# ZooMEISTER/vickers-hardness-Unet

Hardware: AMD Instinct MI355X
Metric: 512x512 images/sec (train fwd+bwd) (higher is better)
Workload: dtype bf16

## Files before the change

### include/vk_unet.h

```cpp
#ifndef VK_UNET_H
#define VK_UNET_H

#include <stddef.h>
#include <stdint.h>

#ifdef __cplusplus
extern "C" {
#endif

#define VK_ABI_VERSION 1
#define VK_STATS_REPLICAS 32

typedef enum { VK_F32 = 0, VK_BF16 = 1, VK_F16 = 2 } vk_dtype;

enum { VK_OK = 0, VK_ERR_ARG = -1, VK_ERR_STATE = -2, VK_ERR_UNSUPPORTED = -3 };

int vk_version(void);
const char* vk_last_error_string(void);
int vk_has_gfx950_code(void);
int vk_probe_mfma_rate(int iters, int waves_per_simd, float* sink, double* flops_out, void* stream);
int vk_set_reserved_cus(int n);
int vk_debug_hold_cus(int workgroups, int threads, int lds_bytes, int microseconds, const void* traffic, size_t traffic_bytes,
                      float* sink, void* stream);

int vk_debug_set_stamp_buffer(void* device_buffer);
int vk_prof_enable(int on);
int vk_prof_collect(char* buf, size_t buflen);


typedef struct {
  const void* ptr;
  int C;
  int up;
  const float* scale;
  const float* shift;
  int relu;
} vk_src;

typedef struct {
  vk_dtype dtype;
  int N, H, W;
  int Ho, Wo;
  int K;
  int R, S, stride, pad;
  int transposed;
  vk_src src0, src1;
} vk_conv_desc;

int vk_conv_fwd(const vk_conv_desc* d, const void* w, void* y, void* y1, int split_k1, int accumulate,
                double* stats, void* stream);

int vk_conv_dgrad_pool2(const vk_conv_desc* d, const void* w, void* y_half, void* y1, int split_k1, int accumulate,
                        void* stream);

int vk_halo_pack(vk_dtype dtype, int rows, int red, const void* src, void* dst, void* stream);
int vk_conv_uses_halo_pack(const vk_conv_desc* d);
int vk_conv_fwd_packed(const vk_conv_desc* d, const void* w_halo, void* y, void* y1, int split_k1, int accumulate, double* stats,
                       void* stream);

#define VK_SPLITK_WORKSPACE_BYTES (32u << 20)
int vk_conv_fwd_splitk(const vk_conv_desc* d, const void* w_halo, void* y, void* workspace, size_t workspace_bytes, void* stream);

typedef struct {
  const void* z;
  const float* scale;
  const float* shift;
  double* sums;
  const void* mask;
  int accumulate;
} vk_bnr;

int vk_conv_dgrad_fused(const vk_conv_desc* d, const void* w, void* y, void* y1, int split_k1, int pool2, const vk_bnr* bnr,
                        void* stream);

int vk_conv1x1_fwd(const vk_conv_desc* d, const void* w, void* y, int accumulate, double* stats, void* stream);
int vk_conv1x1_wgrad(const vk_conv_desc* d, const void* dz, float* dw, void* workspace, size_t workspace_bytes, void* stream);

int vk_stem_fwd(vk_dtype dtype, int N, int H, int W, const void* x4, const void* wp, void* y, double* stats,
                void* stream);

#define VK_WGRAD_WORKSPACE_BYTES (64u << 20)
int vk_conv_wgrad(const vk_conv_desc* d, const void* dz, float* dw, void* workspace, size_t workspace_bytes, void* stream);
#define VK_WGRAD_BATCH_TABLE_BYTES (128u << 10)
int vk_conv_wgrad_batch_supports(const vk_conv_desc* d);
int vk_conv_wgrad_batch(const vk_conv_desc* descs, const void* const* dz, float* const* dw, int n, int workgroups, void* tables,
                        size_t tables_bytes, void* workspace, size_t workspace_bytes, void* stream);
int vk_stem_wgrad(vk_dtype dtype, int N, int H, int W, const void* x4, const void* dz, float* dw_krsc3, void* workspace,
                  size_t workspace_bytes, void* stream);
int vk_stem_wgrad_bn(vk_dtype dtype, int N, int H, int W, const void* x4, const void* g, const void* z, const float* coef_abc,
                     float* dw_krsc3, void* workspace, size_t workspace_bytes, void* stream);
int vk_conv_bwd_onepass(const vk_conv_desc* d_fwd, const void* g, const void* z, const float* coef_abc, const void* w_dgrad, void* y,
                        const vk_bnr* bnr, float* dw, void* workspace, size_t workspace_bytes, void* stream);
int vk_stem_dgrad(vk_dtype dtype, int N, int H, int W, const void* g, const void* z, const float* coef_abc, const float* w_krsc3,
                  float* dx, void* stream);

typedef struct {
  int h, w;
  int src_stride;
  int size;
  int nh, nw;
  int top, left;
  int pad_value;
} vk_letterbox_desc;

int vk_letterbox_preprocess(const vk_letterbox_desc* d, const uint8_t* bgr, float* x_nchw, void* stream);
int vk_letterbox_postprocess_mask(const vk_letterbox_desc* d, const float* logits, float thresh, uint8_t* mask_hw, void* stream);
int vk_letterbox_postprocess_prob(const vk_letterbox_desc* d, const float* logits, float* prob_hw, void* stream);
int vk_letterbox_postprocess_labels(const vk_letterbox_desc* d, int C, const float* logits, uint8_t* labels_hw, void* stream);
int vk_letterbox_postprocess_mask_multi(const vk_letterbox_desc* d, int C, const float* logits, float thresh, uint8_t* masks_chw,
                                        void* stream);
int vk_letterbox_postprocess_prob_multi(const vk_letterbox_desc* d, int C, int mode, const float* logits, float* probs_chw, void* stream);

#define VK_TILE_MAX_ORIGINS 64
#define VK_TILE_MAX_SIDE 4096
#define VK_BLEND_PROB 0
#define VK_BLEND_LOGIT 1
typedef struct {
  int h, w;
  int src_stride;
  int T;
  int overlap;
  int ny, nx;
  int ys[VK_TILE_MAX_ORIGINS], xs[VK_TILE_MAX_ORIGINS];
  int view_mask;
  int pad_value;
  int C;
} vk_tile_desc;

int vk_tile_preprocess(const vk_tile_desc* d, const uint8_t* bgr, float* x, void* stream);
int vk_tile_blend(const vk_tile_desc* d, int mode, const float* logits, float thresh, float* out_chw, uint8_t* mask_chw, void* stream);

typedef struct {
  int h, w;
  float bin_thresh;
  int morph_kernel;
  int open_iter;
  int close_iter;
  int min_area;
  int max_components;
} vk_geom_desc;

typedef struct {
  int label;
  int area;
  int box[8];
  float cx, cy;
  float rw, rh;
  float ux, uy;
  int hull_n;
  int reserved;
  double d1, d2, d_mean;
} vk_geom_det;

int64_t vk_geom_workspace_bytes(const vk_geom_desc* d, int batch);
int vk_geom_minarearect(const vk_geom_desc* d, int batch, const float* prob, uint8_t* clean, vk_geom_det* dets, int* counts,
                        void* workspace, size_t workspace_bytes, void* stream);

typedef struct {
  int label;
  int area;
  int box[8];
  float cx, cy;
  int valid;
  int branch;
  int n_candidates;
  int contour_n;
  int hull_n;
  int flags;
  double quality;
  double d1, d2, d_mean;
} vk_geom_quad;

int vk_geom_quadrilateral(const vk_geom_desc* d, int fit_outset_px, int batch, const float* prob, uint8_t* clean, vk_geom_quad* dets,
                          int* counts, void* workspace, size_t workspace_bytes, void* stream);

typedef struct {
  int d4;
  int rotate;
  float cos_a, sin_a;
  int photo;
  float alpha, beta;
  int blur_ksize;
  float noise_scale;
  uint32_t noise_seed;
  int clahe_limit;
} vk_aug_params;

#define VK_AUG_TABLE_INTS (256 + 4097 + 4097)
size_t vk_augment_workspace_bytes(int n, int size);

int vk_letterbox_u8(const vk_letterbox_desc* d, const uint8_t* bgr, uint8_t* rgb_sq, void* stream);
int vk_letterbox_mask_u8(const vk_letterbox_desc* d, const uint8_t* mask_hw, uint8_t* mask_sq, void* stream);
int vk_augment_batch(int n, int size, int n_items, const uint8_t* images_rgb, const uint8_t* masks, const int* index_dev,
                     const vk_aug_params* params_host, void* params_dev, const int* color_tables, void* workspace,
                     size_t workspace_bytes, float* x, float* y, void* stream);

int vk_input_transform(vk_dtype dtype, int N, int H, int W, const float* x, void* x4, void* stream);

int vk_bn_finalize(int C, int train, const double* stats, double count, const float* gamma, const float* beta,
                   float* running_mean, float* running_var, float eps, float momentum, float* scale, float* shift,
                   float* save_mean, float* save_invstd, void* stream);

int vk_bn_relu_maxpool(vk_dtype dtype, int N, int H, int W, int C, const void* z, const float* scale,
                       const float* shift, void* pooled, uint8_t* argmax, void* stream);
int vk_maxpool_bwd(vk_dtype dtype, int N, int H, int W, int C, const void* dpool, const uint8_t* argmax, void* dy,
                   void* stream);
int vk_maxpool_bwd_bn_reduce(vk_dtype dtype, int N, int H, int W, int C, const void* dpool, const uint8_t* argmax, const void* z,
                             const float* scale, const float* shift, void* dy, double* sums, void* stream);

int vk_bn_add_relu(vk_dtype dtype, size_t pixels, int C, const void* z, const float* scale, const float* shift,
                   const void* res, const float* rscale, const float* rshift, void* out, void* stream);

int vk_bn_bwd_reduce(vk_dtype dtype, size_t pixels, int C, const void* dy, const void* z, int mask_mode,
                     const float* scale, const float* shift, const void* mask_src, double* sums, void* stream);
int vk_bn_bwd_coeffs(int C, const double* sums, double count, const float* gamma, const float* save_mean,
                     const float* save_invstd, float* dgamma, float* dbeta, float* coef_abc, void* stream);
int vk_bn_bwd_apply(vk_dtype dtype, size_t pixels, int C, const void* dy, const void* z, int mask_mode,
                    const float* scale, const float* shift, const void* mask_src, const float* coef_abc, void* dz,
                    void* g_out, int g_accumulate, void* stream);
int vk_bn_bwd_coeffs_frozen(int C, const double* sums, const float* gamma, const float* running_mean, const float* running_invstd,
                            float* dgamma, float* dbeta, float* coef_abc, void* stream);
int vk_bn_bwd_apply_fused(vk_dtype dtype, size_t pixels, int C, const void* dy, const void* z, int mask_mode,
                          const float* scale, const float* shift, const void* mask_src, const double* sums, double count,
                          const float* gamma, const float* save_mean, const float* save_invstd, float* dgamma, float* dbeta,
                          void* dz, void* g_out, int g_accumulate, void* stream);

// ... 178 lines not shown
```

### vickers-hardness-unet_amd/_lib.py

```python
from __future__ import annotations

import ctypes as C
import os
import subprocess
from pathlib import Path

PKG_DIR = Path(__file__).resolve().parent
LIB_PATH = Path(os.environ["VK_LIB"]) if os.environ.get("VK_LIB") else PKG_DIR / "libvkunet.so"
CSRC = PKG_DIR / "csrc"

VK_F32, VK_BF16, VK_F16 = 0, 1, 2
VK_LOSS_BINARY, VK_LOSS_MULTILABEL, VK_LOSS_MULTICLASS = 0, 1, 2
VK_ENC_RESNET18, VK_ENC_RESNET34, VK_ENC_RESNET50 = 18, 34, 50
VK_ADAMW_MAX_GROUPS = 8
VK_NORM_L2, VK_NORM_INF = 0, 1
VK_TILE_MAX_ORIGINS, VK_TILE_MAX_SIDE = 64, 4096
VK_BLEND_PROB, VK_BLEND_LOGIT = 0, 1


class VkError(RuntimeError):
    pass


class vk_src(C.Structure):
    _fields_ = [("ptr", C.c_void_p), ("C", C.c_int), ("up", C.c_int), ("scale", C.c_void_p),
                ("shift", C.c_void_p), ("relu", C.c_int)]


class vk_conv_desc(C.Structure):
    _fields_ = [("dtype", C.c_int), ("N", C.c_int), ("H", C.c_int), ("W", C.c_int), ("Ho", C.c_int),
                ("Wo", C.c_int), ("K", C.c_int), ("R", C.c_int), ("S", C.c_int), ("stride", C.c_int),
                ("pad", C.c_int), ("transposed", C.c_int), ("src0", vk_src), ("src1", vk_src)]


class vk_bnr(C.Structure):
    _fields_ = [("z", C.c_void_p), ("scale", C.c_void_p), ("shift", C.c_void_p), ("sums", C.c_void_p), ("mask", C.c_void_p),
                ("accumulate", C.c_int)]


class vk_letterbox_desc(C.Structure):
    _fields_ = [("h", C.c_int), ("w", C.c_int), ("src_stride", C.c_int), ("size", C.c_int), ("nh", C.c_int),
                ("nw", C.c_int), ("top", C.c_int), ("left", C.c_int), ("pad_value", C.c_int)]


class vk_tile_desc(C.Structure):
    _fields_ = [("h", C.c_int), ("w", C.c_int), ("src_stride", C.c_int), ("T", C.c_int), ("overlap", C.c_int), ("ny", C.c_int),
                ("nx", C.c_int), ("ys", C.c_int * VK_TILE_MAX_ORIGINS), ("xs", C.c_int * VK_TILE_MAX_ORIGINS), ("view_mask", C.c_int),
                ("pad_value", C.c_int), ("C", C.c_int)]


class vk_geom_desc(C.Structure):
    _fields_ = [("h", C.c_int), ("w", C.c_int), ("bin_thresh", C.c_float), ("morph_kernel", C.c_int), ("open_iter", C.c_int),
                ("close_iter", C.c_int), ("min_area", C.c_int), ("max_components", C.c_int)]


class vk_geom_det(C.Structure):
    _fields_ = [("label", C.c_int), ("area", C.c_int), ("box", C.c_int * 8), ("cx", C.c_float), ("cy", C.c_float),
                ("rw", C.c_float), ("rh", C.c_float), ("ux", C.c_float), ("uy", C.c_float), ("hull_n", C.c_int),
                ("reserved", C.c_int), ("d1", C.c_double), ("d2", C.c_double), ("d_mean", C.c_double)]


class vk_geom_quad(C.Structure):
    _fields_ = [("label", C.c_int), ("area", C.c_int), ("box", C.c_int * 8), ("cx", C.c_float), ("cy", C.c_float),
                ("valid", C.c_int), ("branch", C.c_int), ("n_candidates", C.c_int), ("contour_n", C.c_int), ("hull_n", C.c_int),
                ("flags", C.c_int), ("quality", C.c_double), ("d1", C.c_double), ("d2", C.c_double), ("d_mean", C.c_double)]


class vk_aug_params(C.Structure):
    _fields_ = [("d4", C.c_int), ("rotate", C.c_int), ("cos_a", C.c_float), ("sin_a", C.c_float), ("photo", C.c_int),
                ("alpha", C.c_float), ("beta", C.c_float), ("blur_ksize", C.c_int), ("noise_scale", C.c_float),
                ("noise_seed", C.c_uint32), ("clahe_limit", C.c_int)]


class vk_seg_loss_cfg(C.Structure):
    _fields_ = [("struct_size", C.c_uint32), ("mode", C.c_int32), ("terms", C.c_uint32), ("has_ignore", C.c_int32),
                ("ignore_index", C.c_int32), ("w_pix", C.c_float), ("w_focal", C.c_float), ("w_dice", C.c_float),
                ("w_jaccard", C.c_float), ("w_tversky", C.c_float), ("pix_smooth", C.c_float), ("pix_denom_valid", C.c_int32),
                ("has_pos_weight", C.c_int32), ("pos_weight", C.c_float * 16), ("focal_has_alpha", C.c_int32),
                ("focal_alpha", C.c_float), ("focal_gamma", C.c_float),
                ("dice_smooth", C.c_float), ("dice_eps", C.c_float), ("dice_log", C.c_int32), ("dice_classes", C.c_uint32),
                ("jaccard_smooth", C.c_float), ("jaccard_eps", C.c_float), ("jaccard_log", C.c_int32), ("jaccard_classes", C.c_uint32),
                ("tversky_smooth", C.c_float), ("tversky_eps", C.c_float), ("tversky_log", C.c_int32), ("tversky_classes", C.c_uint32),
                ("tversky_alpha", C.c_float), ("tversky_beta", C.c_float), ("tversky_gamma", C.c_float),
                ("w_mcc", C.c_float), ("mcc_eps", C.c_float)]


class vk_lovasz_cfg(C.Structure):
    _fields_ = [("struct_size", C.c_uint32), ("mode", C.c_int32), ("per_image", C.c_int32), ("has_ignore", C.c_int32),
                ("ignore_index", C.c_int32)]


class vk_adamw_group(C.Structure):
    _fields_ = [("lr", C.c_float), ("beta1", C.c_float), ("beta2", C.c_float), ("eps", C.c_float), ("weight_decay", C.c_float)]


class vk_unet_config(C.Structure):
    _fields_ = [("N", C.c_int), ("size", C.c_int), ("dtype", C.c_int), ("training", C.c_int), ("width", C.c_int)]


class vk_tensor_info(C.Structure):
    _fields_ = [("name", C.c_char * 96), ("kind", C.c_int), ("dims", C.c_int * 4), ("ndim", C.c_int),
                ("offset", C.c_int64), ("numel", C.c_int64)]


vp, ci, cf, cd, sz, i64 = C.c_void_p, C.c_int, C.c_float, C.c_double, C.c_size_t, C.c_int64
P = C.POINTER

SIGNATURES = {
    "vk_version": (ci, []),
    "vk_last_error_string": (C.c_char_p, []),
    "vk_has_gfx950_code": (ci, []),
    "vk_probe_mfma_rate": (ci, [ci, ci, vp, P(C.c_double), vp]),
    "vk_set_reserved_cus": (ci, [ci]),
    "vk_debug_hold_cus": (ci, [ci, ci, ci, ci, vp, sz, vp, vp]),
    "vk_debug_set_stamp_buffer": (ci, [vp]),
    "vk_prof_enable": (ci, [ci]),
    "vk_prof_collect": (ci, [C.c_char_p, sz]),
    "vk_conv_fwd": (ci, [P(vk_conv_desc), vp, vp, vp, ci, ci, vp, vp]),
    "vk_conv_dgrad_pool2": (ci, [P(vk_conv_desc), vp, vp, vp, ci, ci, vp]),
    "vk_conv_dgrad_fused": (ci, [P(vk_conv_desc), vp, vp, vp, ci, ci, P(vk_bnr), vp]),
    "vk_head_bwd_fused": (ci, [ci, ci, ci, ci, P(vk_src), vp, vp, vp, vp, vp, P(vk_bnr), vp, sz, vp]),
    "vk_halo_pack": (ci, [ci, ci, ci, vp, vp, vp]),
    "vk_conv_uses_halo_pack": (ci, [P(vk_conv_desc)]),
    "vk_conv_fwd_packed": (ci, [P(vk_conv_desc), vp, vp, vp, ci, ci, vp, vp]),
    "vk_conv_fwd_splitk": (ci, [P(vk_conv_desc), vp, vp, vp, sz, vp]),
    "vk_stem_fwd": (ci, [ci, ci, ci, ci, vp, vp, vp, vp, vp]),
    "vk_conv_wgrad": (ci, [P(vk_conv_desc), vp, vp, vp, sz, vp]),
    "vk_conv1x1_fwd": (ci, [P(vk_conv_desc), vp, vp, ci, vp, vp]),
    "vk_conv1x1_wgrad": (ci, [P(vk_conv_desc), vp, vp, vp, sz, vp]),
    "vk_conv_wgrad_batch_supports": (ci, [P(vk_conv_desc)]),
    "vk_conv_wgrad_batch": (ci, [P(vk_conv_desc), P(vp), P(vp), ci, ci, vp, sz, vp, sz, vp]),
    "vk_stem_wgrad": (ci, [ci, ci, ci, ci, vp, vp, vp, vp, sz, vp]),
    "vk_stem_wgrad_bn": (ci, [ci, ci, ci, ci, vp, vp, vp, vp, vp, vp, sz, vp]),
    "vk_conv_bwd_onepass": (ci, [P(vk_conv_desc), vp, vp, vp, vp, vp, P(vk_bnr), vp, vp, sz, vp]),
    "vk_stem_dgrad": (ci, [ci, ci, ci, ci, vp, vp, vp, vp, vp, vp]),
    "vk_letterbox_preprocess": (ci, [P(vk_letterbox_desc), vp, vp, vp]),
    "vk_letterbox_postprocess_mask": (ci, [P(vk_letterbox_desc), vp, cf, vp, vp]),
    "vk_letterbox_postprocess_prob": (ci, [P(vk_letterbox_desc), vp, vp, vp]),
    "vk_letterbox_postprocess_labels": (ci, [P(vk_letterbox_desc), ci, vp, vp, vp]),
    "vk_letterbox_postprocess_mask_multi": (ci, [P(vk_letterbox_desc), ci, vp, cf, vp, vp]),
    "vk_letterbox_postprocess_prob_multi": (ci, [P(vk_letterbox_desc), ci, ci, vp, vp, vp]),
    "vk_tile_preprocess": (ci, [P(vk_tile_desc), vp, vp, vp]),
    "vk_tile_blend": (ci, [P(vk_tile_desc), ci, vp, cf, vp, vp, vp]),
    "vk_geom_workspace_bytes": (i64, [P(vk_geom_desc), ci]),
    "vk_geom_minarearect": (ci, [P(vk_geom_desc), ci, vp, vp, vp, vp, vp, sz, vp]),
    "vk_geom_quadrilateral": (ci, [P(vk_geom_desc), ci, ci, vp, vp, vp, vp, vp, sz, vp]),
    "vk_letterbox_u8": (ci, [P(vk_letterbox_desc), vp, vp, vp]),
    "vk_letterbox_mask_u8": (ci, [P(vk_letterbox_desc), vp, vp, vp]),
    "vk_augment_workspace_bytes": (C.c_size_t, [ci, ci]),
    "vk_augment_batch": (ci, [ci, ci, ci, vp, vp, vp, P(vk_aug_params), vp, vp, vp, C.c_size_t, vp, vp, vp]),
    "vk_input_transform": (ci, [ci, ci, ci, ci, vp, vp, vp]),
    "vk_bn_finalize": (ci, [ci, ci, vp, cd, vp, vp, vp, vp, cf, cf, vp, vp, vp, vp, vp]),
    "vk_bn_relu_maxpool": (ci, [ci, ci, ci, ci, ci, vp, vp, vp, vp, vp, vp]),
    "vk_maxpool_bwd": (ci, [ci, ci, ci, ci, ci, vp, vp, vp, vp]),
    "vk_maxpool_bwd_bn_reduce": (ci, [ci, ci, ci, ci, ci, vp, vp, vp, vp, vp, vp, vp, vp]),
    "vk_bn_add_relu": (ci, [ci, sz, ci, vp, vp, vp, vp, vp, vp, vp, vp]),
    "vk_bn_bwd_reduce": (ci, [ci, sz, ci, vp, vp, ci, vp, vp, vp, vp, vp]),
    "vk_bn_bwd_coeffs": (ci, [ci, vp, cd, vp, vp, vp, vp, vp, vp, vp]),
    "vk_bn_bwd_coeffs_frozen": (ci, [ci, vp, vp, vp, vp, vp, vp, vp, vp]),
    "vk_bn_bwd_apply": (ci, [ci, sz, ci, vp, vp, ci, vp, vp, vp, vp, vp, vp, ci, vp]),
    "vk_bn_bwd_apply_fused": (ci, [ci, sz, ci, vp, vp, ci, vp, vp, vp, vp, cd, vp, vp, vp, vp, vp, vp, vp, ci, vp]),
    "vk_upsample2x_bwd": (ci, [ci, ci, ci, ci, ci, vp, vp, ci, vp]),
    "vk_head_fwd": (ci, [ci, ci, ci, ci, P(vk_src), vp, vp, vp, vp]),
    "vk_dec4_tail_eval": (ci, [ci, ci, ci, ci, P(vk_src), vp, vp, vp, vp, vp, vp, vp, vp, vp, vp]),
    "vk_head_bwd": (ci, [ci, ci, ci, ci, P(vk_src), vp, vp, vp, vp, vp, vp, sz, vp]),
    "vk_bce_dice_loss": (ci, [sz, vp, vp, vp, vp, vp, cf, cf, cf, vp]),
    "vk_head_fwd_multi": (ci, [ci, ci, ci, ci, ci, P(vk_src), vp, vp, vp, vp]),
    "vk_head_multi_workspace_bytes": (sz, [ci]),
    "vk_head_bwd_multi": (ci, [ci, ci, ci, ci, ci, P(vk_src), vp, vp, vp, vp, vp, P(vk_bnr), vp, sz, vp]),
    "vk_multi_loss_workspace_bytes": (sz, [ci, ci, ci]),
    "vk_multilabel_loss": (ci, [ci, ci, ci, vp, vp, vp, sz, vp, vp, cf, cf, cf, vp]),
    "vk_multiclass_loss": (ci, [ci, ci, ci, vp, vp, vp, sz, vp, vp, cf, cf, cf, vp]),
    "vk_seg_loss_cfg_size": (sz, []),
    "vk_seg_loss_workspace_bytes": (sz, [ci, ci, ci]),
    "vk_seg_loss": (ci, [P(vk_seg_loss_cfg), ci, ci, ci, vp, vp, vp, sz, vp, vp, cf, vp]),
    "vk_lovasz_cfg_size": (sz, []),
    "vk_lovasz_workspace_bytes": (sz, [P(vk_lovasz_cfg), ci, ci, ci]),
    "vk_lovasz_loss": (ci, [P(vk_lovasz_cfg), ci, ci, ci, vp, vp, vp, sz, vp, vp, cf, ci, vp]),
    "vk_lovasz_flat_workspace_bytes": (sz, [ci, i64]),
    "vk_lovasz_flat": (ci, [vp, vp, ci, i64, vp, sz, vp, vp, vp, vp]),
    "vk_seg_metrics_workspace_bytes": (C.c_size_t, [ci]),
    "vk_seg_metrics": (ci, [ci, sz, vp, vp, ci, cf, cf, vp, sz, vp, vp]),
    "vk_seg_metrics_multi_workspace_bytes": (sz, [ci, ci]),
    "vk_seg_metrics_multi": (ci, [ci, ci, ci, sz, vp, vp, ci, cf, cf, vp, sz, vp, vp, vp, vp]),
    "vk_adamw_step": (ci, [sz, vp, vp, vp, vp, cf, cf, cf, cf, cf, ci, cf, vp, vp, ci, vp]),
    "vk_amp_check_inf": (ci, [sz, vp, vp, vp]),
    "vk_amp_unscale_check": (ci, [sz, vp, vp, vp, vp]),
    "vk_adamw_step_amp": (ci, [sz, vp, vp, vp, vp, cf, cf, cf, cf, cf, vp, cf, vp, vp, vp, vp, ci, vp]),
    "vk_adamw_segment_blocks": (ci, [ci, P(i64), P(C.c_int32), ci]),
    "vk_adamw_step_amp_segments": (ci, [ci, vp, ci, vp, vp, vp, vp, vp, cf, cf, cf, cf, cf, vp, cf, vp, vp, vp, vp]),
    "vk_adamw_step_groups": (ci, [ci, vp, vp, ci, vp, vp, vp, vp, vp, ci, P(vk_adamw_group), vp, cf, vp, vp, vp, vp, vp]),
    "vk_grad_norm_segments": (ci, [ci, vp, ci, vp, vp, ci, cf, cf, vp, vp, vp]),
    "vk_unet_create": (ci, [P(vk_unet_config), P(vp)]),
    "vk_unet_create_ex": (ci, [P(vk_unet_config), ci, P(vp)]),
    "vk_unet_num_classes": (ci, [vp]),
    "vk_unet_create_enc": (ci, [P(vk_unet_config), ci, ci, P(vp)]),
    "vk_unet_encoder": (ci, [vp]),
    "vk_unet_destroy": (None, [vp]),
    "vk_unet_set_side_stream": (ci, [vp, ci]),
    "vk_unet_num_tensors": (ci, [vp]),
    "vk_unet_tensor_info": (ci, [vp, ci, P(vk_tensor_info)]),
    "vk_unet_param_numel": (i64, [vp]),
    "vk_unet_buffer_numel": (i64, [vp]),
    "vk_unet_workspace_bytes": (i64, [vp]),
    "vk_unet_num_buckets": (ci, [vp]),
    "vk_unet_bucket_range": (ci, [vp, ci, P(i64), P(i64)]),
    "vk_unet_bind": (ci, [vp, vp, vp, vp, vp, vp, sz]),
    "vk_unet_refresh_weights": (ci, [vp, vp]),
    "vk_unet_forward": (ci, [vp, vp, vp, ci, vp]),
    "vk_unet_loss": (ci, [vp, vp, vp, vp, cf, cf, cf, vp]),
    "vk_unet_loss_ex": (ci, [vp, ci, vp, vp, vp, cf, cf, cf, vp]),
    "vk_unet_loss_cfg": (ci, [vp, P(vk_seg_loss_cfg), vp, vp, vp, cf, vp]),
    "vk_unet_loss_lovasz": (ci, [vp, P(vk_seg_loss_cfg), P(vk_lovasz_cfg), cf, vp, vp, vp, sz, vp, cf, vp]),
    "vk_unet_backward": (ci, [vp, vp, ci, ci, vp]),
    "vk_unet_set_trainable": (ci, [vp, P(C.c_uint8), ci]),
    "vk_unet_set_bn_frozen": (ci, [vp, P(C.c_uint8), ci]),
    "vk_unet_set_input_grad": (ci, [vp, vp]),
    "vk_unet_zero_grad": (ci, [vp, vp]),
    "vk_unet_debug_tensor": (ci, [vp, C.c_char_p, P(vp), P(ci * 4)]),
    "vk_comm_unique_id": (ci, [vp]),
    "vk_comm_init": (ci, [ci, ci, vp, P(vp)]),
    "vk_comm_world": (ci, [vp]),
    "vk_allreduce_bucket": (ci, [vp, vp, sz, vp]),
    "vk_comm_broadcast": (ci, [vp, vp, sz, ci, vp]),
    "vk_comm_destroy": (ci, [vp]),
}

_lib = None


def build(force: bool = False, verbose: bool = False) -> Path:
    srcs = list(CSRC.glob("*.hip")) + list(CSRC.glob("*.h")) + [PKG_DIR.parent / "include" / "vk_unet.h"]
    if not force and LIB_PATH.exists() and all(LIB_PATH.stat().st_mtime >= s.stat().st_mtime for s in srcs):
        return LIB_PATH
    hipcc = os.environ.get("HIPCC", "/opt/rocm/bin/hipcc")
    if not Path(hipcc).exists():
        raise VkError(f"hipcc not found at {hipcc}; cannot build libvkunet.so")
    cmd = ["make", "-C", str(CSRC), f"-j{min(4, os.cpu_count() or 1)}", f"HIPCC={hipcc}"]
    r = subprocess.run(cmd, capture_output=True, text=True)
    if verbose:
        print(r.stdout[-2000:], r.stderr[-2000:])
    if r.returncode != 0 or not LIB_PATH.exists():
        raise VkError("building libvkunet.so failed:\n" + r.stdout[-3000:] + r.stderr[-3000:])
    return LIB_PATH


def lib():
    global _lib
    if _lib is not None:
        return _lib
    if not LIB_PATH.exists():
        raise VkError(f"{LIB_PATH} is missing: build it with __graft_entry__.build() "
                      f"(make -C {CSRC}); this package has no CPU fallback")
    try:
        L = C.CDLL(str(LIB_PATH))
    except OSError as e:
        raise VkError(f"cannot load {LIB_PATH}: {e}") from e
    for name, (res, args) in SIGNATURES.items():
        fn = getattr(L, name, None)
        if fn is None:
            raise VkError(f"{LIB_PATH} does not export {name}")
        fn.restype = res
        fn.argtypes = args
    if L.vk_version() != 1:
        raise VkError("libvkunet.so ABI version mismatch")
    _lib = L
    return L


def check(rc: int, what: str = "") -> None:
    if rc != 0:
        msg = lib().vk_last_error_string().decode(errors="replace")
        kind = "argument/state error" if rc < 0 else f"hipError {rc}"
        raise VkError(f"{what or 'libvkunet'}: {kind}: {msg}")


def dtype_code(dt) -> int:
    import torch
# ... 21 lines not shown
```

### vickers-hardness-unet_amd/csrc/conv_halo.hip

```cpp
#include <stdlib.h>
#include <string.h>

#include <string>
#include <type_traits>

#include "vk_common.h"

#ifdef VK_STAMP
#define VK_T(var) { __builtin_amdgcn_sched_barrier(0); const unsigned long long t_ = __builtin_amdgcn_s_memtime(); __builtin_amdgcn_s_waitcnt(0xC07F); __builtin_amdgcn_sched_barrier(0); var = t_; }
#else
#define VK_T(var)
#endif

namespace vk {

struct HaloSrc {
  const void* ptr;
  const float* scale;
  const float* shift;
  int C, up, relu;
  uint32_t bytes;
};

#ifndef VK_EPI_BATCH_READS
#define VK_EPI_BATCH_READS 1
#endif
#ifndef VK_COLP_DEFER_STATS
#define VK_COLP_DEFER_STATS 1
#endif
#ifndef VK_COLQ_ILV
#define VK_COLQ_ILV 1
#endif
#ifndef VK_COLQ_DIAG
#define VK_COLQ_DIAG 0
#endif
#ifndef VK_COLQ_PRE
#define VK_COLQ_PRE 1
#endif
struct HaloParams {
  HaloSrc s0, s1;
  const void* w;
  uint32_t w_bytes;
  void* y0;
  void* y1;
  int ld0, ld1, split;
  double* stats;
  int N, H, W, K, C, flip, accumulate, pool2;
  int Hi, Wi;
  int tiles_x, tiles_y, nchunks;
  unsigned long long* stamps;
  int kyn;
  int ksplit;
  size_t slab_bytes;
  float* slab;
  int dbg;
  const void* bnr_z;
  const float* bnr_scale;
  const float* bnr_shift;
  double* bnr_sums;
  const void* bnr_mask;
};

template <typename T, int TH, int BN, int WGM, int WGN>
struct HaloCfg {
  using Tr = ElemTraits<T>;
  static constexpr int EB = Tr::kBytes;
  static constexpr int VE = Tr::kVec;
  static constexpr int CK = 64 / EB;
  static constexpr int HW_ = 18, HH = TH + 2, HPIX = HH * HW_;
  static constexpr int APS = 96;
  static constexpr int A_BYTES = HPIX * APS;
  static constexpr int B_BYTES = 3 * BN * 64;
  static constexpr int NPV = (HPIX * 4 + 255) / 256;
  static constexpr int NBV = (3 * BN * 4 + 255) / 256;
  static constexpr int BM = TH * 16;
  static constexpr int WR = TH / WGM;
  static constexpr int WCH = BN / WGN;
  static constexpr int TP = WR, TC = WCH / 16;
  static constexpr int ESB = BN * EB + 16;
  static constexpr int EVPR = BN / VE;
  static constexpr int ERPP = 256 / EVPR;
  static constexpr int EPASS = BM / ERPP;
  static constexpr int RED_OFF = BM * ESB;
  static constexpr int MAIN = A_BYTES + 2 * B_BYTES;
  static constexpr int ESLOTS = (BN / VE > 16) ? 4 * 4 / (BN / VE / 16) : 4 * 4;
  static constexpr int EPI = RED_OFF + ESLOTS * BN * 2 * 4;
  static constexpr int SMEM = MAIN > EPI ? MAIN : EPI;
  static_assert(WGM * WGN == 4 && TH % WGM == 0 && BN % (16 * WGN) == 0, "wave layout");
  static_assert(EPASS >= 1, "epilogue mapping");
  static_assert(SMEM <= 160 * 1024, "main-loop / epilogue LDS image exceeds the 160 KiB of a CU");
};

__device__ __forceinline__ int swz(int row) { return ((row >> 2) & 1) << 1; }

__device__ __forceinline__ int halo_group(int tid) {
  const int g = tid >> 2;
  return (g & ~3) | ((g & 1) << 1) | ((g >> 1) & 1);
}


template <typename T, int TH, int BN, int TP, int TC, int NT = 256, bool PRE = false, int OS = 1>
__device__ __forceinline__ void halo_epilogue(char* smem, f32x4_t (&acc)[TC][TP], const HaloParams& p, int n, int y0, int x0, int n0,
                                              int wrow0, int wch0, int py = 0, int px = 0, double* defer = nullptr) {
  using Tr = ElemTraits<T>;
  constexpr int EB = Tr::kBytes, VE = Tr::kVec;
  constexpr int BM = TH * 16;
  constexpr int ESB = BN * EB + 16;
  constexpr int EVPR = BN / VE, ERPP = NT / EVPR, EPASS = BM / ERPP, NW = NT / 64;
  constexpr int RED_OFF = BM * ESB;
  static_assert(BM % ERPP == 0 && EVPR <= 64, "epilogue mapping");
  const int tid = threadIdx.x, lane = tid & 63, wave = tid >> 6;
  const int li = lane & 15, kg = lane >> 4;

  const int e_row = tid / EVPR;
  const int e_vec = (EVPR == 16 && EB == 2) ? (((tid & 15) + ((e_row & 1) ? 15 : 0)) & 15) : tid % EVPR;
  const int col0 = n0 + e_vec * VE;
  const bool col_ok = col0 < p.K;
  char* yb = (char*)p.y0;
  int ld = p.ld0, colx = col0;
  bool first_part = true;
  if (p.split > 0 && col0 >= p.split) { yb = (char*)p.y1; ld = p.ld1; colx = col0 - p.split; first_part = false; }
  float s1[VE], s2[VE];
#pragma unroll
  for (int j = 0; j < VE; ++j) { s1[j] = 0.f; s2[j] = 0.f; }
  const bool bnr = p.bnr_z != nullptr && first_part && col_ok;
  const bool ext_mask = p.bnr_mask != nullptr;
  float bsc[VE], bsh[VE];
  if (bnr && !ext_mask) {
#pragma unroll
    for (int j = 0; j < VE; ++j) { bsc[j] = p.bnr_scale[colx + j]; bsh[j] = p.bnr_shift[colx + j]; }
  }
  auto finish = [&](float (&f)[VE], size_t elem_off, const u32x4_t* pre_old, const u32x4_t* pre_z, const u32x4_t* pre_m = nullptr) {
    u32x4_t* gp = reinterpret_cast<u32x4_t*>(yb + elem_off * EB);
    if (p.accumulate) {
      float o[VE];
      Vec16<T>::unpack(pre_old ? *pre_old : *gp, o);
#pragma unroll
      for (int j = 0; j < VE; ++j) f[j] += o[j];
    }
    u32x4_t v = Vec16<T>::pack(f);
    Vec16<T>::unpack(v, f);
    if (bnr) {
      float zf[VE];
      Vec16<T>::unpack(pre_z ? *pre_z : *reinterpret_cast<const u32x4_t*>((const char*)p.bnr_z + elem_off * EB), zf);
      if (ext_mask) {
        float mf[VE];
        Vec16<T>::unpack(pre_m ? *pre_m : *reinterpret_cast<const u32x4_t*>((const char*)p.bnr_mask + elem_off * EB), mf);
#pragma unroll
        for (int j = 0; j < VE; ++j)
          if (!(mf[j] > 0.f)) f[j] = 0.f;
      } else {
#pragma unroll
        for (int j = 0; j < VE; ++j)
          if (!(fmaf(zf[j], bsc[j], bsh[j]) > 0.f)) f[j] = 0.f;
      }
#pragma unroll
      for (int j = 0; j < VE; ++j) {
        s1[j] += f[j];
        s2[j] += f[j] * zf[j];
      }
      v = Vec16<T>::pack(f);
    } else {
#pragma unroll
      for (int j = 0; j < VE; ++j) { s1[j] += f[j]; s2[j] += f[j] * f[j]; }
    }
    *gp = v;
  };
  constexpr bool PRE_M = PRE && NT == 512;
  u32x4_t oldv[PRE ? EPASS : 1], zv[PRE ? EPASS : 1], mv[PRE_M ? EPASS : 1];
  constexpr bool EARLY = PRE && NT == 512;
  auto request_pre = [&]() {
    if (!(PRE && (p.accumulate || bnr) && !(p.pool2 && first_part))) return;
#pragma unroll
    for (int ps = 0; ps < (PRE ? EPASS : 0); ++ps) {
      const int row = e_row + ps * ERPP;
      const int y = OS * (y0 + (row >> 4)) + py, x = OS * (x0 + (row & 15)) + px;
      oldv[ps] = u32x4_t{0, 0, 0, 0};
      zv[ps] = u32x4_t{0, 0, 0, 0};
      if (PRE_M) mv[ps] = u32x4_t{0, 0, 0, 0};
      if (y < p.H && x < p.W && col_ok) {
        const size_t eoff = (((size_t)n * p.H + y) * p.W + x) * ld + colx;
        if (p.accumulate) oldv[ps] = *reinterpret_cast<const u32x4_t*>(yb + eoff * EB);
        if (bnr) zv[ps] = *reinterpret_cast<const u32x4_t*>((const char*)p.bnr_z + eoff * EB);
        if (PRE_M && bnr && ext_mask) mv[ps] = *reinterpret_cast<const u32x4_t*>((const char*)p.bnr_mask + eoff * EB);
      }
    }
  };
  if (EARLY) request_pre();
#pragma unroll
  for (int a = 0; a < TC; ++a)
#pragma unroll
    for (int b = 0; b < TP; ++b) {
      const int ch = wch0 + a * 16 + kg * 4;
      const int px = (wrow0 + b) * 16 + li;
      char* dst = smem + px * ESB + ch * EB;
      if (EB == 4) {
        *reinterpret_cast<f32x4_t*>(dst) = acc[a][b];
      } else {
        float f[8] = {acc[a][b][0], acc[a][b][1], acc[a][b][2], acc[a][b][3], 0.f, 0.f, 0.f, 0.f};
        const u32x4_t pk = Vec16<T>::pack(f);
        *reinterpret_cast<u32x2_t*>(dst) = u32x2_t{pk[0], pk[1]};
      }
    }
  __syncthreads();
  if (!EARLY) request_pre();

  if (p.pool2 && first_part) {
    const int Hh = p.H >> 1, Wh = p.W >> 1;
    for (int pr = e_row; pr < (TH / 2) * 8; pr += ERPP) {
      const int py = pr >> 3, px = pr & 7;
      const int y = (y0 >> 1) + py, x = (x0 >> 1) + px;
      if (y < Hh && x < Wh && col_ok) {
        float f[VE];
// ... 173 lines not shown
    const bool first = c < p.s0.C;
    const HaloSrc& sd = first ? p.s0 : p.s1;
    const int cl = (first ? c : c - p.s0.C) + hv * VE;
    aff = sd.scale != nullptr;
    relu = sd.relu != 0;
    if (aff) {
#pragma unroll
      for (int j = 0; j < VE; j += 4) {
        const f32x4_t s4 = *reinterpret_cast<const f32x4_t*>(sd.scale + cl + j);
        const f32x4_t h4 = *reinterpret_cast<const f32x4_t*>(sd.shift + cl + j);
#pragma unroll
        for (int e = 0; e < 4; ++e) { sc[j + e] = s4[e]; sh[j + e] = h4[e]; }
      }
    }
    const bool up = sd.up != 0;
#pragma unroll
    for (int i = 0; i < NPV; ++i) {
      const int pix = up ? h_half[i] : h_full[i];
      const uint32_t off = (uint32_t)(pix * sd.C + cl) * (uint32_t)EB;
      if (first) areg[i] = buf_load16(rs0, pix >= 0 ? off : kOOB);
      else areg[i] = buf_load16(rs1, pix >= 0 ? off : kOOB);
    }
  };

  auto store_halo = [&]() {
#pragma unroll
    for (int i = 0; i < NPV; ++i) {
      const int hp = hgrp + i * 64;
      if (hp >= HPIX) continue;
      u32x4_t v = areg[i];
      if (aff) {
        v = AffineRelu<T>::run(v, sc, sh, relu);
        if (h_full[i] < 0) v = u32x4_t{0, 0, 0, 0};
      }
      *reinterpret_cast<u32x4_t*>(Abuf + hp * APS + hv * 16) = v;
    }
  };

  auto load_b = [&](u32x4_t (&breg)[NBV], int stage) {
    const int cc = stage / 3, r = stage - cc * 3;
#pragma unroll
    for (int i = 0; i < NBV; ++i) {
      const int tap = p.flip ? 8 - (3 * r + b_s[i]) : 3 * r + b_s[i];
      const uint32_t base = (uint32_t)(cc * 9 + tap) * slab_bytes + (uint32_t)n0 * 64u;
      breg[i] = buf_load16(rsw, b_toff[i] >= 0 ? base + (uint32_t)b_toff[i] : kOOB);
    }
  };
  auto store_b = [&](const u32x4_t (&breg)[NBV], int buf) {
    char* B = Bbuf + buf * Cfg::B_BYTES;
#pragma unroll
    for (int i = 0; i < NBV; ++i)
      if (b_toff[i] >= 0) *reinterpret_cast<u32x4_t*>(B + b_s[i] * (BN * 64) + b_toff[i]) = breg[i];
  };

  const int wrow0 = (wave / WGN) * Cfg::WR;
  const int wch0 = (wave % WGN) * Cfg::WCH;
  f32x4_t acc[TC][TP];
#pragma unroll
  for (int a = 0; a < TC; ++a)
#pragma unroll
    for (int b = 0; b < TP; ++b) acc[a][b] = f32x4_t{0.f, 0.f, 0.f, 0.f};
  const int li = lane & 15, kg = lane >> 4;
  const char* const a_lane = Abuf + (wrow0 * 18 + li) * APS + kg * 16;
  const int b_lane = (wch0 + li) * 64 + ((kg ^ swz(li)) << 4);

  auto compute = [&](int bbuf, int r) {
    const char* A = a_lane + r * (18 * APS);
    const char* B = Bbuf + bbuf * Cfg::B_BYTES + b_lane;
    u32x4_t wf[2][TC], xf[2][TP];
#pragma unroll
    for (int a = 0; a < TC; ++a) wf[0][a] = *reinterpret_cast<const u32x4_t*>(B + (a * 16) * 64);
#pragma unroll
    for (int b = 0; b < TP; ++b) xf[0][b] = *reinterpret_cast<const u32x4_t*>(A + (b * 18) * APS);
#pragma unroll
    for (int s = 0; s < 3; ++s) {
      if (s < 2) {
#pragma unroll
        for (int a = 0; a < TC; ++a) wf[(s + 1) & 1][a] = *reinterpret_cast<const u32x4_t*>(B + ((s + 1) * BN + a * 16) * 64);
#pragma unroll
        for (int b = 0; b < TP; ++b) xf[(s + 1) & 1][b] = *reinterpret_cast<const u32x4_t*>(A + (b * 18 + s + 1) * APS);
      }
#pragma unroll
      for (int a = 0; a < TC; ++a)
#pragma unroll
        for (int b = 0; b < TP; ++b) acc[a][b] = Mma<T>::run(wf[s & 1][a], xf[s & 1][b], acc[a][b]);
    }
    constexpr int NR = TC + TP, NM = TC * TP * (sizeof(T) == 4 ? 4 : 1);
    __builtin_amdgcn_sched_group_barrier(0x100, NR, 0);
    __builtin_amdgcn_sched_group_barrier(0x100, NR, 0);
    __builtin_amdgcn_sched_group_barrier(0x008, NM, 0);
    __builtin_amdgcn_sched_group_barrier(0x100, NR, 0);
    __builtin_amdgcn_sched_group_barrier(0x008, NM, 0);
    __builtin_amdgcn_sched_group_barrier(0x008, NM, 0);
  };

#ifdef VK_STAMP
  unsigned long long t_begin;
  VK_T(t_begin)
#endif
  const int nst = p.nchunks * 3;
  load_halo(0);
  load_b(breg0, 0);
  store_halo();
  store_b(breg0, 0);
  if (nst > 1) load_b(breg1, 1);
  __syncthreads();

#ifdef VK_STAMP
  unsigned long long tk_load = 0, tk_comp = 0, tk_store = 0, tk_bar = 0;
#endif
  auto stage = [&](int st, u32x4_t (&ld_regs)[NBV], const u32x4_t (&st_regs)[NBV]) {
    const int cc = st / 3, r = st - cc * 3;
    const bool next_chunk = cc + 1 < p.nchunks;
#ifdef VK_STAMP
    unsigned long long t0, t1, t2, t3, t4;
#endif
    VK_T(t0)
    if (st + 2 < nst) load_b(ld_regs, st + 2);
    if (r == 0 && next_chunk) load_halo(cc + 1);
    VK_T(t1)
    compute(st & 1, r);
    VK_T(t2)
    if (r == 2 && next_chunk) {
      __syncthreads();
      store_halo();
    }
    if (st + 1 < nst) store_b(st_regs, (st + 1) & 1);
    VK_T(t3)
    __syncthreads();
    VK_T(t4)
#ifdef VK_STAMP
    tk_load += t1 - t0; tk_comp += t2 - t1; tk_store += t3 - t2; tk_bar += t4 - t3;
#endif
  };
  for (int st = 0; st < nst; st += 2) {
    stage(st, breg0, breg1);
    if (st + 1 < nst) stage(st + 1, breg1, breg0);
  }

#ifdef VK_STAMP
  unsigned long long te0, te1;
  VK_T(te0)
#endif
  halo_epilogue<T, TH, BN, TP, TC>(smem, acc, p, n, y0, x0, n0, wrow0, wch0);
#ifdef VK_STAMP
  VK_T(te1)
  if (p.stamps && lane == 0) {
    unsigned long long* o = p.stamps + ((size_t)(blockIdx.y * gridDim.x + blockIdx.x) * 4 + wave) * 8;
    o[0] = tk_load; o[1] = tk_comp; o[2] = tk_store; o[3] = tk_bar; o[4] = te1 - te0; o[5] = te0 - t_begin; o[6] = te1 - t_begin; o[7] = nst;
  }
#endif
}

template <typename T, int TH, int BN, int WGM, int WGN, bool ADB, int STR = 1>
struct ColCfg {
  using Tr = ElemTraits<T>;
  static constexpr int EB = Tr::kBytes;
  static constexpr int VE = Tr::kVec;
  static constexpr int CK = 64 / EB;
  static constexpr int NW = WGM * WGN, NT = 64 * NW;
  static constexpr int HH = STR == 1 ? TH + 2 : 2 * TH + 1;
  static constexpr int HWI = STR == 1 ? 18 : 33;
  static constexpr int RS = STR == 1 ? 18 : 34;
  static constexpr int HPIX = HH * HWI;
  static constexpr int APS = 96;
  static constexpr int A_BYTES = HH * RS * APS;
  static constexpr int NA = ADB ? 2 : 1;
  static constexpr int B_BYTES = 3 * BN * 64;
  static constexpr int NPV = (HPIX * 4 + NT - 1) / NT;
  static constexpr int NPIECE = 3 * BN / 16;
  static constexpr int BM = TH * 16;
  static constexpr int TP = TH / WGM, TC = BN / WGN / 16;
  static constexpr int NX = STR * (TP - 1) + 3;
  static constexpr int ESB = BN * EB + 16;
  static constexpr int NB = (BN <= 64 && STR == 1) ? 3 : 2;
  static constexpr int MAIN = NA * A_BYTES + NB * B_BYTES;
  static constexpr int ESLOTS = (BN / VE > 16) ? NW * 4 / (BN / VE / 16) : NW * 4;
  static constexpr int EPI = BM * ESB + ESLOTS * BN * 2 * 4;
  static constexpr int SMEM = MAIN > EPI ? MAIN : EPI;
  static_assert(TH % WGM == 0 && BN % (16 * WGN) == 0 && (NW == 4 || NW == 8), "wave layout");
  static_assert(STR == 1 || STR == 2, "stride");
  static_assert(SMEM <= 160 * 1024, "main-loop / epilogue LDS image exceeds the 160 KiB of a CU");
  static_assert(EPI >= BM * ESB + ESLOTS * BN * 8, "epilogue partial-sum slots must fit behind the output tile");
};

template <typename T, int TH, int BN, int WGM, int WGN, bool ADB, int MINW, int STR = 1>
__global__ __launch_bounds__(64 * WGM * WGN, MINW) void conv3x3_col_kernel(const HaloParams p) {
  using Cfg = ColCfg<T, TH, BN, WGM, WGN, ADB, STR>;
  constexpr int EB = Cfg::EB, VE = Cfg::VE, CK = Cfg::CK, HPIX = Cfg::HPIX, NPV = Cfg::NPV, NT = Cfg::NT, NW = Cfg::NW;
  constexpr int TP = Cfg::TP, TC = Cfg::TC, APS = Cfg::APS, NPIECE = Cfg::NPIECE, RS = Cfg::RS, HWI = Cfg::HWI, NX = Cfg::NX;
  typedef __attribute__((address_space(3))) void lds_void;

  extern __shared__ __attribute__((aligned(16))) char smem[];
  char* const Abuf = smem;
  char* const Bbuf = smem + Cfg::NA * Cfg::A_BYTES;
  const int tid = threadIdx.x, lane = tid & 63;
  const int wave = __builtin_amdgcn_readfirstlane(tid >> 6);

  int bt = blockIdx.x;
  int ky = blockIdx.y;
  if (p.kyn > 0) {
    const int j = bt >> 3;
    ky = j % p.kyn;
    bt = (bt & 7) * (int)((gridDim.x / p.kyn) >> 3) + j / p.kyn;
  } else if (p.kyn < 0) {
    const int kn = -p.kyn, xcd = bt & 7;
    ky = xcd % kn;
    bt = (xcd / kn) * (int)(gridDim.x >> 3) + (bt >> 3);
  } else if ((gridDim.x & 7) == 0) {
    bt = (bt & 7) * (int)(gridDim.x >> 3) + (bt >> 3);
  }
  const int tx = bt % p.tiles_x;
  bt /= p.tiles_x;
  const int ty = bt % p.tiles_y;
  const int n = bt / p.tiles_y;
  const int y0 = ty * TH, x0 = tx * 16;
  const int n0 = ky * BN;

  const __amdgpu_buffer_rsrc_t rs0 = make_rsrc(p.s0.ptr, p.s0.bytes);
  const __amdgpu_buffer_rsrc_t rs1 = make_rsrc(p.s1.ptr ? p.s1.ptr : p.s0.ptr, p.s1.ptr ? p.s1.bytes : 0u);
  const __amdgpu_buffer_rsrc_t rsw = make_rsrc(p.w, p.w_bytes);

  const int hv = tid & 3;
  const int hgrp = halo_group(tid);
  int h_full[NPV], h_half[NPV];
  const int Hh = p.Hi >> 1, Wh = p.Wi >> 1;
#pragma unroll
  for (int i = 0; i < NPV; ++i) {
    const int hp = hgrp + i * (NT / 4);
    const int hy = hp / HWI, hx = hp - hy * HWI;
    const int y = STR * y0 - 1 + hy, x = STR * x0 - 1 + hx;
    const bool ok = hp < HPIX && (unsigned)y < (unsigned)p.Hi && (unsigned)x < (unsigned)p.Wi;
    h_full[i] = ok ? (n * p.Hi + y) * p.Wi + x : -1;
    h_half[i] = ok ? (n * Hh + (y >> 1)) * Wh + (x >> 1) : -1;
  }
  u32x4_t areg[NPV];
  float sc[VE], sh[VE];
  bool aff = false, relu = false;

  auto load_halo = [&](int cc) {
    const int c = cc * CK;
    const bool first = c < p.s0.C;
    const HaloSrc& sd = first ? p.s0 : p.s1;
    const int cl = (first ? c : c - p.s0.C) + hv * VE;
    aff = sd.scale != nullptr;
    relu = sd.relu != 0;
    if (aff) {
#pragma unroll
      for (int j = 0; j < VE; j += 4) {
        const f32x4_t s4 = *reinterpret_cast<const f32x4_t*>(sd.scale + cl + j);
        const f32x4_t h4 = *reinterpret_cast<const f32x4_t*>(sd.shift + cl + j);
#pragma unroll
        for (int e = 0; e < 4; ++e) { sc[j + e] = s4[e]; sh[j + e] = h4[e]; }
      }
    }
    const bool up = STR == 1 && sd.up != 0;
#pragma unroll
    for (int i = 0; i < NPV; ++i) {
      const int pix = up ? h_half[i] : h_full[i];
      const uint32_t off = (uint32_t)(pix * sd.C + cl) * (uint32_t)EB;
      if (first) areg[i] = buf_load16(rs0, pix >= 0 ? off : kOOB);
      else areg[i] = buf_load16(rs1, pix >= 0 ? off : kOOB);
    }
  };
  auto store_halo = [&](char* A) {
#pragma unroll
    for (int i = 0; i < NPV; ++i) {
      const int hp = hgrp + i * (NT / 4);
      if (hp >= HPIX) continue;
      u32x4_t v = areg[i];
      if (aff) {
        v = AffineRelu<T>::run(v, sc, sh, relu);
        if (h_full[i] < 0) v = u32x4_t{0, 0, 0, 0};
      }
      int slot = hp;
      if (STR == 2) {
        const int hy = hp / HWI, hx = hp - hy * HWI;
        slot = hy * RS + (hx & 1) * 17 + (hx >> 1);
      }
      *reinterpret_cast<u32x4_t*>(A + slot * APS + hv * 16) = v;
    }
  };

  const uint32_t slab_bytes = (uint32_t)p.K * 64u;
  const uint32_t lane16 = (uint32_t)lane * 16u;
  auto dma_b = [&](int cc, int s, int buf) {
#pragma unroll
    for (int i = 0; i < (NPIECE + NW - 1) / NW; ++i) {
      const int pc = wave + i * NW;
      if (NPIECE % NW == 0 || pc < NPIECE) {
        const int r = pc / (BN / 16), sub = pc - r * (BN / 16);
        const int tap = p.flip ? 8 - (3 * r + s) : 3 * r + s;
        const uint32_t goff = (uint32_t)(cc * 9 + tap) * slab_bytes + (uint32_t)(n0 + sub * 16) * 64u;
        char* dst = Bbuf + buf * Cfg::B_BYTES + (r * BN + sub * 16) * 64;
        __builtin_amdgcn_raw_ptr_buffer_load_lds(rsw, (lds_void*)dst, 16, lane16, goff, 0, 0);
      }
    }
  };

  const int wrow0 = (wave / WGN) * TP;
  const int wch0 = (wave % WGN) * (TC * 16);
  f32x4_t acc[TC][TP];
#pragma unroll
  for (int a = 0; a < TC; ++a)
#pragma unroll
    for (int b = 0; b < TP; ++b) acc[a][b] = f32x4_t{0.f, 0.f, 0.f, 0.f};
  const int li = lane & 15, kg = lane >> 4;
  const int a_lane = (STR * wrow0 * RS + li) * APS + kg * 16;
  const int b_lane = (wch0 + li) * 64 + ((kg ^ swz(li)) << 4);

  auto compute = [&](const char* A, const char* B) {
    u32x4_t X[NX], W[3][TC];
#pragma unroll
    for (int h = 0; h < NX; ++h) X[h] = *reinterpret_cast<const u32x4_t*>(A + h * (RS * APS));
#pragma unroll
    for (int r = 0; r < 3; ++r)
#pragma unroll
      for (int a = 0; a < TC; ++a) W[r][a] = *reinterpret_cast<const u32x4_t*>(B + (r * BN + a * 16) * 64);
#pragma unroll
    for (int r = 0; r < 3; ++r)
#pragma unroll
      for (int a = 0; a < TC; ++a)
#pragma unroll
        for (int b = 0; b < TP; ++b) acc[a][b] = Mma<T>::run(W[r][a], X[STR * b + r], acc[a][b]);
    constexpr int NM = TC * TP * (sizeof(T) == 4 ? 4 : 1);
    __builtin_amdgcn_sched_group_barrier(0x100, NX + TC, 0);
    __builtin_amdgcn_sched_group_barrier(0x100, TC, 0);
    __builtin_amdgcn_sched_group_barrier(0x008, NM, 0);
    __builtin_amdgcn_sched_group_barrier(0x100, TC, 0);
    __builtin_amdgcn_sched_group_barrier(0x008, NM, 0);
    __builtin_amdgcn_sched_group_barrier(0x008, NM, 0);
  };

#ifdef VK_STAMP
  unsigned long long t_begin, t_pro, tk_load = 0, tk_comp = 0, tk_store = 0, tk_bar = 0;
  VK_T(t_begin)
#endif
  const int ksp = p.ksplit > 1 ? p.ksplit : 1;
  const int c_begin = (int)((long)p.nchunks * blockIdx.z / ksp), c_end = (int)((long)p.nchunks * (blockIdx.z + 1) / ksp);
  load_halo(c_begin);
  dma_b(c_begin, 0, 0);
  const bool one_chunk = Cfg::NB == 3 && c_end - c_begin == 1 && !p.dbg;
  if (one_chunk) {
    dma_b(c_begin, 1, 1);
    dma_b(c_begin, 2, 2);
  }
  store_halo(Abuf);
  __syncthreads();
  VK_T(t_pro)

  int st = 0;
  if (one_chunk) {
    const char* A = Abuf + a_lane;
#pragma unroll
    for (int s = 0; s < 3; ++s) compute(A + (STR == 1 ? s : (s & 1) * 17 + (s >> 1)) * APS, Bbuf + s * Cfg::B_BYTES + b_lane);
    __syncthreads();
    st = 3;
  }
  for (int cc = c_begin; cc < c_end && !one_chunk; ++cc) {
    const bool next_chunk = cc + 1 < c_end;
    const char* A = Abuf + (ADB ? ((cc - c_begin) & 1) * Cfg::A_BYTES : 0) + a_lane;
    char* const Anext = Abuf + (ADB ? ((cc - c_begin + 1) & 1) * Cfg::A_BYTES : 0);
#pragma unroll
    for (int s = 0; s < 3; ++s, ++st) {
#ifdef VK_STAMP
      unsigned long long t0, t1, t2, t3, t4;
#endif
      VK_T(t0)
      if (!(p.dbg & 2)) {
        if (s < 2) dma_b(cc, s + 1, (st + 1) & 1);
        else if (next_chunk) dma_b(cc + 1, 0, (st + 1) & 1);
      }
      if (s == 0 && next_chunk && !(p.dbg & 4)) load_halo(cc + 1);
      VK_T(t1)
      compute(A + (STR == 1 ? s : (s & 1) * 17 + (s >> 1)) * APS, Bbuf + (st & 1) * Cfg::B_BYTES + b_lane);
      VK_T(t2)
      if (ADB) {
        if (s == 1 && next_chunk && !(p.dbg & 4)) store_halo(Anext);
      } else {
        if (s == 2 && next_chunk && !(p.dbg & 4)) {
          __syncthreads();
          store_halo(Anext);
        }
      }
      VK_T(t3)
      if (!(p.dbg & 8)) __syncthreads();
      VK_T(t4)
#ifdef VK_STAMP
      tk_load += t1 - t0; tk_comp += t2 - t1; tk_store += t3 - t2; tk_bar += t4 - t3;
#endif
    }
  }
#ifdef VK_STAMP
  unsigned long long te0, te1;
  VK_T(te0)
#endif
  if (p.ksplit > 1) {
    float* sl = p.slab + (size_t)blockIdx.z * ((size_t)p.N * p.H * p.W * p.K);
#pragma unroll
    for (int a = 0; a < TC; ++a)
#pragma unroll
      for (int b = 0; b < TP; ++b) {
        const int y = y0 + wrow0 + b, x = x0 + li, ch = n0 + wch0 + a * 16 + kg * 4;
        if (y < p.H && x < p.W && ch < p.K) *reinterpret_cast<f32x4_t*>(sl + (((size_t)n * p.H + y) * p.W + x) * p.K + ch) = acc[a][b];
      }
    return;
  }
  halo_epilogue<T, TH, BN, TP, TC, NT, (BN <= 64 && TH == 16)>(smem, acc, p, n, y0, x0, n0, wrow0, wch0);
#ifdef VK_STAMP
  VK_T(te1)
  if (p.stamps && lane == 0) {
    unsigned long long* o = p.stamps + ((size_t)(blockIdx.y * gridDim.x + blockIdx.x) * NW + wave) * 8;
    o[0] = tk_load; o[1] = tk_comp; o[2] = tk_store; o[3] = tk_bar; o[4] = te1 - te0; o[5] = t_pro - t_begin; o[6] = te1 - t_begin; o[7] = st;
  }
#endif
}

template <typename T, int TH, int BN, int WGM, int WGN>
struct S2dCfg {
  using Tr = ElemTraits<T>;
  static constexpr int EB = Tr::kBytes, VE = Tr::kVec, CK = 64 / EB;
  static constexpr int NW = WGM * WGN, NT = 64 * NW;
  static constexpr int HH = TH + 1, RS = 17, HPIX = HH * RS, APS = 96;
  static constexpr int A_BYTES = HPIX * APS;
  static constexpr int B_BYTES = 3 * BN * 64;
  static constexpr int NPV = (HPIX * 4 + NT - 1) / NT;
  static constexpr int NPIECE = 3 * BN / 16;
  static constexpr int BM = TH * 16;
  static constexpr int TP = TH / WGM, TC = BN / WGN / 16;
  static constexpr int ESB = BN * EB + 16;
  static constexpr int MAIN = 2 * A_BYTES + 2 * B_BYTES;
  static constexpr int ESLOTS = (BN / VE > 16) ? NW * 4 / (BN / VE / 16) : NW * 4;
  static constexpr int EPI = BM * ESB + ESLOTS * BN * 2 * 4;
  static constexpr int SMEM = MAIN > EPI ? MAIN : EPI;
  static_assert(TH % WGM == 0 && BN % (16 * WGN) == 0 && NW == 8, "wave layout");
  static_assert(4 * TP * TC <= 32, "accumulator budget (four parity classes)");
  static_assert(SMEM <= 160 * 1024, "LDS image exceeds the 160 KiB of a CU");
};

template <typename T, int TH, int BN, int WGM, int WGN>
__global__ __launch_bounds__(64 * WGM * WGN, 1) void conv3x3_s2dg_kernel(const HaloParams p) {
  using Cfg = S2dCfg<T, TH, BN, WGM, WGN>;
  constexpr int EB = Cfg::EB, VE = Cfg::VE, CK = Cfg::CK, HPIX = Cfg::HPIX, NPV = Cfg::NPV, NT = Cfg::NT, NW = Cfg::NW;
  constexpr int TP = Cfg::TP, TC = Cfg::TC, APS = Cfg::APS, NPIECE = Cfg::NPIECE, RS = Cfg::RS;
  typedef __attribute__((address_space(3))) void lds_void;

  extern __shared__ __attribute__((aligned(16))) char smem[];
  char* const Abuf = smem;
  char* const Bbuf = smem + 2 * Cfg::A_BYTES;
  const int tid = threadIdx.x, lane = tid & 63;
  const int wave = __builtin_amdgcn_readfirstlane(tid >> 6);

  int bt = blockIdx.x;
  const int ky = blockIdx.y;
  if ((gridDim.x & 7) == 0) bt = (bt & 7) * (int)(gridDim.x >> 3) + (bt >> 3);
  const int tx = bt % p.tiles_x;
  bt /= p.tiles_x;
  const int ty = bt % p.tiles_y;
  const int n = bt / p.tiles_y;
  const int y0 = ty * TH, x0 = tx * 16;
  const int n0 = ky * BN;

  const __amdgpu_buffer_rsrc_t rs0 = make_rsrc(p.s0.ptr, p.s0.bytes);
  const __amdgpu_buffer_rsrc_t rsw = make_rsrc(p.w, p.w_bytes);

  const int hv = tid & 3;
  const int hgrp = halo_group(tid);
  int h_full[NPV];
#pragma unroll
  for (int i = 0; i < NPV; ++i) {
    const int hp = hgrp + i * (NT / 4);
    const int hy = hp / RS, hx = hp - hy * RS;
    const int y = y0 + hy, x = x0 + hx;
    const bool ok = hp < HPIX && y < p.Hi && x < p.Wi;
    h_full[i] = ok ? (n * p.Hi + y) * p.Wi + x : -1;
  }
  u32x4_t areg[NPV];
  auto load_halo = [&](int cc) {
    const int cl = cc * CK + hv * VE;
#pragma unroll
    for (int i = 0; i < NPV; ++i) {
      const uint32_t off = (uint32_t)(h_full[i] * p.s0.C + cl) * (uint32_t)EB;
      areg[i] = buf_load16(rs0, h_full[i] >= 0 ? off : kOOB);
    }
  };
  auto store_halo = [&](char* A) {
#pragma unroll
    for (int i = 0; i < NPV; ++i) {
      const int hp = hgrp + i * (NT / 4);
      if (hp < HPIX) *reinterpret_cast<u32x4_t*>(A + hp * APS + hv * 16) = areg[i];
    }
  };
  const uint32_t slab_bytes = (uint32_t)p.K * 64u;
  const uint32_t lane16 = (uint32_t)lane * 16u;
  auto dma_b = [&](int cc, int s, int buf) {
#pragma unroll
    for (int i = 0; i < (NPIECE + NW - 1) / NW; ++i) {
      const int pc = wave + i * NW;
      if (NPIECE % NW == 0 || pc < NPIECE) {
        const int r = pc / (BN / 16), sub = pc - r * (BN / 16);
        const uint32_t goff = (uint32_t)(cc * 9 + 3 * r + s) * slab_bytes + (uint32_t)(n0 + sub * 16) * 64u;
        char* dst = Bbuf + buf * Cfg::B_BYTES + (r * BN + sub * 16) * 64;
        __builtin_amdgcn_raw_ptr_buffer_load_lds(rsw, (lds_void*)dst, 16, lane16, goff, 0, 0);
      }
    }
  };

  const int wrow0 = (wave / WGN) * TP;
  const int wch0 = (wave % WGN) * (TC * 16);
  f32x4_t acc[4][TC][TP];
#pragma unroll
  for (int q = 0; q < 4; ++q)
#pragma unroll
    for (int a = 0; a < TC; ++a)
#pragma unroll
      for (int b = 0; b < TP; ++b) acc[q][a][b] = f32x4_t{0.f, 0.f, 0.f, 0.f};
  const int li = lane & 15, kg = lane >> 4;
  const int a_lane = (wrow0 * RS + li) * APS + kg * 16;
  const int b_lane = (wch0 + li) * 64 + ((kg ^ swz(li)) << 4);

  auto compute = [&](const char* A, const char* B, auto s_c) {
    constexpr int s = decltype(s_c)::value;
    u32x4_t X[TP + 1], W[3][TC];
#pragma unroll
    for (int h = 0; h < TP + 1; ++h) X[h] = *reinterpret_cast<const u32x4_t*>(A + ((s == 0 ? 1 : 0) + h * RS) * APS);
#pragma unroll
    for (int r = 0; r < 3; ++r)
#pragma unroll
      for (int a = 0; a < TC; ++a) W[r][a] = *reinterpret_cast<const u32x4_t*>(B + (r * BN + a * 16) * 64);
#pragma unroll
    for (int r = 0; r < 3; ++r) {
      constexpr int px = s != 1 ? 1 : 0;
      const int q = (r != 1 ? 2 : 0) + px, di = r == 0 ? 1 : 0;
#pragma unroll
      for (int a = 0; a < TC; ++a)
#pragma unroll
        for (int b = 0; b < TP; ++b) acc[q][a][b] = Mma<T>::run(W[r][a], X[b + di], acc[q][a][b]);
    }
  };

  load_halo(0);
  dma_b(0, 0, 0);
  store_halo(Abuf);
  __syncthreads();
  int st = 0;
  for (int cc = 0; cc < p.nchunks; ++cc) {
    const bool next_chunk = cc + 1 < p.nchunks;
    const char* A = Abuf + (cc & 1) * Cfg::A_BYTES + a_lane;
    char* const Anext = Abuf + ((cc + 1) & 1) * Cfg::A_BYTES;
    dma_b(cc, 1, (st + 1) & 1);
    if (next_chunk) load_halo(cc + 1);
    compute(A, Bbuf + (st & 1) * Cfg::B_BYTES + b_lane, std::integral_constant<int, 0>{});
    __syncthreads();
    ++st;
    dma_b(cc, 2, (st + 1) & 1);
    compute(A, Bbuf + (st & 1) * Cfg::B_BYTES + b_lane, std::integral_constant<int, 1>{});
    if (next_chunk) store_halo(Anext);
    __syncthreads();
    ++st;
    if (next_chunk) dma_b(cc + 1, 0, (st + 1) & 1);
    compute(A, Bbuf + (st & 1) * Cfg::B_BYTES + b_lane, std::integral_constant<int, 2>{});
    __syncthreads();
    ++st;
  }
#pragma unroll
  for (int q = 0; q < 4; ++q) {
    if (q) __syncthreads();
    halo_epilogue<T, TH, BN, TP, TC, NT, false, 2>(smem, acc[q], p, n, y0, x0, n0, wrow0, wch0, q >> 1, q & 1);
  }
}

template <typename T, int TH, int BN, int WGM, int WGN>
struct ColqCfg : ColCfg<T, TH, BN, WGM, WGN, true> {
  using Base = ColCfg<T, TH, BN, WGM, WGN, true>;
  static constexpr int MAIN = 2 * Base::A_BYTES + 3 * Base::B_BYTES;
  static constexpr int SMEM = MAIN > Base::EPI ? MAIN : Base::EPI;
  static constexpr int DMAW = Base::NPIECE / Base::NW;
  static_assert(Base::NPIECE % Base::NW == 0, "every wave must issue the same number of weight DMAs per stage (partial vmcnt wait)");
  static_assert(DMAW >= 1 && DMAW <= 15, "vmcnt immediate");
  static_assert(SMEM <= 160 * 1024, "LDS image exceeds the 160 KiB of a CU");
};

template <typename T, int TH, int BN, int WGM, int WGN>
__global__ __launch_bounds__(64 * WGM * WGN, 1) void conv3x3_colq_kernel(const HaloParams p) {
  using Cfg = ColqCfg<T, TH, BN, WGM, WGN>;
  constexpr int EB = Cfg::EB, VE = Cfg::VE, CK = Cfg::CK, HPIX = Cfg::HPIX, NPV = Cfg::NPV, NT = Cfg::NT, NW = Cfg::NW;
  constexpr int TP = Cfg::TP, TC = Cfg::TC, APS = Cfg::APS, NPIECE = Cfg::NPIECE;
  typedef __attribute__((address_space(3))) void lds_void;

  extern __shared__ __attribute__((aligned(16))) char smem[];
  char* const Abuf = smem;
  char* const Bbuf = smem + 2 * Cfg::A_BYTES;
  const int tid = threadIdx.x, lane = tid & 63;
  const int wave = __builtin_amdgcn_readfirstlane(tid >> 6);

  int bt = blockIdx.x;
  int ky = blockIdx.y;
  if (p.kyn > 0) {
    const int j = bt >> 3;
    ky = j % p.kyn;
    bt = (bt & 7) * (int)((gridDim.x / p.kyn) >> 3) + j / p.kyn;
  } else if (p.kyn < 0) {
    const int kn = -p.kyn, xcd = bt & 7;
    ky = xcd % kn;
    bt = (xcd / kn) * (int)(gridDim.x >> 3) + (bt >> 3);
  } else if ((gridDim.x & 7) == 0) {
    bt = (bt & 7) * (int)(gridDim.x >> 3) + (bt >> 3);
  }
  const int tx = bt % p.tiles_x;
  bt /= p.tiles_x;
  const int ty = bt % p.tiles_y;
  const int n = bt / p.tiles_y;
  const int y0 = ty * TH, x0 = tx * 16;
  const int n0 = ky * BN;

  const __amdgpu_buffer_rsrc_t rs0 = make_rsrc(p.s0.ptr, p.s0.bytes);
  const __amdgpu_buffer_rsrc_t rs1 = make_rsrc(p.s1.ptr ? p.s1.ptr : p.s0.ptr, p.s1.ptr ? p.s1.bytes : 0u);
  const __amdgpu_buffer_rsrc_t rsw = make_rsrc(p.w, p.w_bytes);

  const int hv = tid & 3;
  const int hgrp = halo_group(tid);
  int h_full[NPV], h_half[NPV];
  const int Hh = p.H >> 1, Wh = p.W >> 1;
#pragma unroll
  for (int i = 0; i < NPV; ++i) {
    const int hp = hgrp + i * (NT / 4);
    const int hy = hp / 18, hx = hp - hy * 18;
    const int y = y0 - 1 + hy, x = x0 - 1 + hx;
    const bool ok = hp < HPIX && (unsigned)y < (unsigned)p.H && (unsigned)x < (unsigned)p.W;
    h_full[i] = ok ? (n * p.H + y) * p.W + x : -1;
    h_half[i] = ok ? (n * Hh + (y >> 1)) * Wh + (x >> 1) : -1;
  }
  u32x4_t areg[NPV];
  float sc[VE], sh[VE];
  bool aff = false, relu = false;

  auto load_halo = [&](int cc) {
    const int c = cc * CK;
    const bool first = c < p.s0.C;
    const HaloSrc& sd = first ? p.s0 : p.s1;
    const int cl = (first ? c : c - p.s0.C) + hv * VE;
    aff = sd.scale != nullptr;
    relu = sd.relu != 0;
    if (aff) {
#pragma unroll
      for (int j = 0; j < VE; j += 4) {
        const f32x4_t s4 = *reinterpret_cast<const f32x4_t*>(sd.scale + cl + j);
        const f32x4_t h4 = *reinterpret_cast<const f32x4_t*>(sd.shift + cl + j);
#pragma unroll
        for (int e = 0; e < 4; ++e) { sc[j + e] = s4[e]; sh[j + e] = h4[e]; }
      }
    }
    const bool up = sd.up != 0;
#pragma unroll
    for (int i = 0; i < NPV; ++i) {
      const int pix = up ? h_half[i] : h_full[i];
      const uint32_t off = (uint32_t)(pix * sd.C + cl) * (uint32_t)EB;
      if (first) areg[i] = buf_load16(rs0, pix >= 0 ? off : kOOB);
      else areg[i] = buf_load16(rs1, pix >= 0 ? off : kOOB);
    }
  };
  auto store_halo = [&](char* A) {
#pragma unroll
    for (int i = 0; i < NPV; ++i) {
      const int hp = hgrp + i * (NT / 4);
      if (hp >= HPIX) continue;
      u32x4_t v = areg[i];
      if (aff) {
        v = (p.dbg & 32) ? AffineReluScalar<T>::run(v, sc, sh, relu) : AffineRelu<T>::run(v, sc, sh, relu);
        if (h_full[i] < 0) v = u32x4_t{0, 0, 0, 0};
      }
      *reinterpret_cast<u32x4_t*>(A + hp * APS + hv * 16) = v;
    }
  };

  const uint32_t slab_bytes = (uint32_t)p.K * 64u;
  const uint32_t lane16 = (uint32_t)lane * 16u;
  auto dma_b = [&](int cc, int s, uint32_t oob = 0u) {
#pragma unroll
    for (int i = 0; i < ((VK_COLQ_DIAG & 1) ? 1 : Cfg::DMAW); ++i) {
      const int pc = wave + i * NW;
      const int r = pc / (BN / 16), sub = pc - r * (BN / 16);
      const int tap = p.flip ? 8 - (3 * r + s) : 3 * r + s;
      const uint32_t goff = (uint32_t)(cc * 9 + tap) * slab_bytes + (uint32_t)(n0 + sub * 16) * 64u;
      char* dst = Bbuf + s * Cfg::B_BYTES + (r * BN + sub * 16) * 64;
      __builtin_amdgcn_raw_ptr_buffer_load_lds(rsw, (lds_void*)dst, 16, lane16 | oob, goff, 0, 0);
    }
  };


  auto dma_one = [&](int cc, int s, int i, uint32_t oob) {
    const int pc = wave + i * NW;
    const int r = pc / (BN / 16), sub = pc - r * (BN / 16);
    const int tap = p.flip ? 8 - (3 * r + s) : 3 * r + s;
    const uint32_t goff = (uint32_t)(cc * 9 + tap) * slab_bytes + (uint32_t)(n0 + sub * 16) * 64u;
    char* dst = Bbuf + s * Cfg::B_BYTES + (r * BN + sub * 16) * 64;
    __builtin_amdgcn_raw_ptr_buffer_load_lds(rsw, (lds_void*)dst, 16, lane16 | oob, goff, 0, 0);
  };

  const int wrow0 = (wave / WGN) * TP;
  const int wch0 = (wave % WGN) * (TC * 16);
  f32x4_t acc[TC][TP];
#pragma unroll
// ... 1389 lines not shown
  dim3 grid((unsigned)(p.N * p.tiles_y * p.tiles_x), (unsigned)((p.K + BN - 1) / BN), 1);
  const size_t out_elems = (size_t)p.N * p.H * p.W * p.K;
  int ks = 1;
  if (p.slab && !p.stats && !p.bnr_z && !p.accumulate && !p.pool2 && p.split == 0 && !getenv("VK_NO_SPLITK")) {
    const long wgs = (long)grid.x * grid.y;
    const char* force = getenv("VK_SPLITK");
    ks = force ? atoi(force) : (wgs < 128 ? (int)(256 / wgs) : 1);
    if (ks > p.nchunks / 2) ks = p.nchunks / 2;
    if (ks > 32) ks = 32;
    while (ks > 1 && (size_t)ks * out_elems * sizeof(float) > p.slab_bytes) --ks;
    if (ks < 2) ks = 1;
  }
  p.ksplit = ks;
  grid.z = (unsigned)ks;
  p.kyn = 0;
  if (ks == 1 && grid.y > 1 && (grid.x & 7) == 0 && !getenv("VK_COL_NO_KYFAST")) {
    p.kyn = (int)grid.y;
    grid.x *= grid.y;
    grid.y = 1;
    const char* km = getenv("VK_COL_KYMODE");
    const bool wst = km ? km[0] == 'w' : (size_t)p.w_bytes >= (3u << 20);
    if (PIPE && wst && 8 % p.kyn == 0 && (grid.x / 8) * (8 / p.kyn) * p.kyn == grid.x) p.kyn = -p.kyn;
  }
  static bool attr_done = false;
  if (!attr_done && Cfg::SMEM > 64 * 1024) {
    VK_CHECK_HIP(hipFuncSetAttribute(kernel, hipFuncAttributeMaxDynamicSharedMemorySize, Cfg::SMEM));
    attr_done = true;
  }
  {
    static const std::string tag_f = std::string(PIPE == 2 ? "cols_" : PIPE == 1 ? "colq_" : "col_") + (sizeof(T) == 4 ? "f32" : "16b") + "_t" + std::to_string(TH) + "_bn" +
                                     std::to_string(BN) + "_w" + std::to_string(WGM * WGN) + (STR == 2 ? "_s2" : "");
    static const std::string tag_d = tag_f + "_dgrad";
    const double macs = (double)p.N * p.H * p.W * p.K * 9.0 * p.C;
    const double bytes = ((double)p.N * ((double)p.Hi * p.Wi * p.C + (double)p.H * p.W * p.K) + 9.0 * p.K * p.C) * sizeof(T);
    const std::string& btag = p.flip ? tag_d : tag_f;
    const std::string dtag = getenv("VK_PROF_DETAIL") ? btag + ":H" + std::to_string(p.H) + "_K" + std::to_string(p.K) + "_C" + std::to_string(p.C) : btag;
    vkh::ProfScope ps(dtag.c_str(), st, 2.0 * macs, bytes);
    void* args[] = {(void*)&p};
    VK_CHECK_HIP(hipLaunchKernel(kernel, grid, dim3(Cfg::NT), args, Cfg::SMEM, st));
  }
  if (ks > 1) {
    vkh::ProfScope ps("splitk_reduce", st, 0.0, (double)out_elems * (4.0 * ks + sizeof(T)));
    hipLaunchKernelGGL(k_splitk_reduce<T>, dim3((unsigned)((out_elems / 4 + 255) / 256)), dim3(256), 0, st, out_elems / 4, ks, p.slab, (T*)p.y0);
  }
  VK_CHECK_HIP(hipGetLastError());
  return VK_OK;
}

template <typename T, int TH, int BN, int WGM, int WGN, int MINW>
static int launch_colp(HaloParams p, hipStream_t st) {
  using Cfg = ColCfg<T, TH, BN, WGM, WGN, false>;
  p.tiles_x = (p.W + 15) / 16;
  p.tiles_y = (p.H + TH - 1) / TH;
  p.kyn = (p.K + BN - 1) / BN;
  p.ksplit = 1;
  const long total = (long)p.N * p.tiles_y * p.tiles_x * p.kyn;
  int per_cu = (160 * 1024) / Cfg::SMEM;
  if (per_cu > 4) per_cu = 4;
  if (per_cu < 1) per_cu = 1;
  long g = 256L * per_cu;
  if (const char* e = getenv("VK_COL_PERSIST_GRID")) g = atol(e) > 0 ? atol(e) : g;
  if (g > total) g = total;
  static bool attr_done = false;
  if (!attr_done && Cfg::SMEM > 64 * 1024) {
    VK_CHECK_HIP(hipFuncSetAttribute((const void*)conv3x3_colp_kernel<T, TH, BN, WGM, WGN, MINW>,
                                     hipFuncAttributeMaxDynamicSharedMemorySize, Cfg::SMEM));
    attr_done = true;
  }
  {
    static const std::string tag_f = std::string("col_") + (sizeof(T) == 4 ? "f32" : "16b") + "_t" + std::to_string(TH) + "_bn" + std::to_string(BN) +
                                     "_w" + std::to_string(WGM * WGN);
    static const std::string tag_d = tag_f + "_dgrad";
    const double macs = (double)p.N * p.H * p.W * p.K * 9.0 * p.C;
    const double bytes = ((double)p.N * p.H * p.W * (p.C + p.K) + 9.0 * p.K * p.C) * sizeof(T);
    const std::string& btag = p.flip ? tag_d : tag_f;
    const std::string dtag = getenv("VK_PROF_DETAIL") ? btag + ":H" + std::to_string(p.H) + "_K" + std::to_string(p.K) + "_C" + std::to_string(p.C) : btag;
    vkh::ProfScope ps(dtag.c_str(), st, 2.0 * macs, bytes);
    hipLaunchKernelGGL((conv3x3_colp_kernel<T, TH, BN, WGM, WGN, MINW>), dim3((unsigned)g), dim3(Cfg::NT), Cfg::SMEM, st, p);
  }
  VK_CHECK_HIP(hipGetLastError());
  return VK_OK;
}

template <typename T, int BN>
static int launch_small(const HaloParams& p, hipStream_t st) {
  const long total = (long)p.N * ((p.H + 15) / 16) * ((p.W + 15) / 16) * ((p.K + BN - 1) / BN);
  const char* pe = getenv("VK_COL_PERSIST");
  const long min_tiles = pe ? (atol(pe) == 0 ? -1 : atol(pe)) : (BN == 64 ? 1024 : -1);
  const bool splitk_wanted = p.slab && !p.stats && !p.bnr_z && !p.accumulate && !p.pool2 && p.split == 0 && total < 128;
  if (min_tiles > 0 && !splitk_wanted && total >= min_tiles) return launch_colp<T, 16, BN, 4, 1, 2>(p, st);
  return launch_col<T, 16, BN, 4, 1, false, 2>(p, st);
}

template <typename T>
static int col_select(const HaloParams& p, hipStream_t st) {
  const char* alt_s = getenv("VK_COL_ALT");
  const int alt = alt_s ? atoi(alt_s) : 0;
  const long tiles16 = (long)p.N * ((p.H + 15) / 16) * ((p.W + 15) / 16);
  if (p.K >= 128) {
    const long kt = (p.K + 127) / 128;
    if (alt == 1) return launch_col<T, 16, 128, 2, 2, true, 1>(p, st);
    if (alt == 8 || (alt == 0 && p.nchunks <= 2 && p.K % 128 != 0) || (alt == 0 && p.nchunks == 1)) return launch_small<T, 64>(p, st);
    if (alt == 3 || (alt != 2 && alt != 7 && p.nchunks <= 2)) return launch_col<T, 8, 128, 2, 2, false, 2>(p, st);
    const char* const pipe_s = getenv("VK_COL_PIPE");
    const int pipe = pipe_s ? atoi(pipe_s) : 1;
    if (alt == 7 || (alt != 2 && tiles16 * kt < 256))
      return pipe == 2 ? launch_col<T, 8, 128, 2, 4, true, 1, 2>(p, st)
             : pipe    ? launch_col<T, 8, 128, 2, 4, true, 1, 1>(p, st) : launch_col<T, 8, 128, 2, 4, true, 2>(p, st);
    if (alt == 9) return launch_col<T, 16, 128, 2, 4, true, 1, 1>(p, st);
    return pipe == 2 ? launch_col<T, 16, 128, 4, 2, true, 1, 2>(p, st)
           : pipe    ? launch_col<T, 16, 128, 4, 2, true, 1, 1>(p, st) : launch_col<T, 16, 128, 4, 2, true, 2>(p, st);
  }
  if (p.K >= 64) return launch_small<T, 64>(p, st);
  if (p.K >= 32) return launch_small<T, 32>(p, st);
  return launch_small<T, 16>(p, st);
}

template <typename T>
static int halo_select(const HaloParams& p, hipStream_t st) {
  const bool old_loop = getenv("VK_HALO_ROWSTAGED") != nullptr;
  if (!old_loop) return col_select<T>(p, st);
  const long tiles8 = (long)p.N * ((p.H + 7) / 8) * ((p.W + 15) / 16);
  const long tiles16 = (long)p.N * ((p.H + 15) / 16) * ((p.W + 15) / 16);
  if (p.K >= 128) {
    if (tiles8 * ((p.K + 127) / 128) >= 512) return launch_halo<T, 8, 128, 2, 2>(p, st);
    return launch_halo<T, 8, 64, 2, 2>(p, st);
  }
  if (p.K >= 64) {
    if (tiles16 >= 1024) return launch_halo<T, 16, 64, 4, 1>(p, st);
    return launch_halo<T, 8, 64, 2, 2>(p, st);
  }
  if (p.K >= 32) return launch_halo<T, 16, 32, 4, 1>(p, st);
  return launch_halo<T, 16, 16, 4, 1>(p, st);
}

template <typename T, int BN>
static int launch_c16(HaloParams p, hipStream_t st) {
  using Cfg = C16Cfg<T, BN>;
  p.tiles_x = (p.W + 15) / 16;
  p.tiles_y = (p.H + 15) / 16;
  dim3 grid((unsigned)(p.N * p.tiles_y * p.tiles_x), (unsigned)((p.K + BN - 1) / BN), 1);
  {
    static const std::string tag_f = std::string("c16_16b_bn") + std::to_string(BN);
    static const std::string tag_d = tag_f + "_dgrad";
    const std::string& btag = p.flip ? tag_d : tag_f;
    const double bytes = ((double)p.N * p.H * p.W * (16.0 + p.K * (p.pool2 ? 0.25 : 1.0)) + 9.0 * p.K * 16.0) * 2.0;
    vkh::ProfScope ps(btag.c_str(), st, 2.0 * (double)p.N * p.H * p.W * p.K * 144.0, bytes);
    hipLaunchKernelGGL((conv3x3_c16_kernel<T, BN>), grid, dim3(256), Cfg::SMEM, st, p);
  }
  VK_CHECK_HIP(hipGetLastError());
  return VK_OK;
}

template <typename T, int BN>
static int launch_s2dg(HaloParams p, hipStream_t st) {
  using Cfg = S2dCfg<T, 8, BN, 4, 2>;
  p.tiles_x = (p.Wi + 15) / 16;
  p.tiles_y = (p.Hi + 7) / 8;
  dim3 grid((unsigned)(p.N * p.tiles_y * p.tiles_x), (unsigned)((p.K + BN - 1) / BN), 1);
  static bool attr_done = false;
  if (!attr_done && Cfg::SMEM > 64 * 1024) {
    VK_CHECK_HIP(hipFuncSetAttribute((const void*)conv3x3_s2dg_kernel<T, 8, BN, 4, 2>, hipFuncAttributeMaxDynamicSharedMemorySize, Cfg::SMEM));
    attr_done = true;
  }
  {
    static const std::string tag = std::string("s2dg_") + (sizeof(T) == 4 ? "f32" : "16b") + "_bn" + std::to_string(BN);
    const std::string dtag = getenv("VK_PROF_DETAIL") ? tag + ":H" + std::to_string(p.H) + "_K" + std::to_string(p.K) + "_C" + std::to_string(p.C) : tag;
    const double bytes = ((double)p.N * ((double)p.Hi * p.Wi * p.C + (double)p.H * p.W * p.K * (p.accumulate ? 2.0 : 1.0)) + 9.0 * p.K * p.C) * sizeof(T);
    vkh::ProfScope ps(dtag.c_str(), st, 2.0 * (double)p.N * p.Hi * p.Wi * p.K * 9.0 * p.C, bytes);
    hipLaunchKernelGGL((conv3x3_s2dg_kernel<T, 8, BN, 4, 2>), grid, dim3(Cfg::NT), Cfg::SMEM, st, p);
  }
  VK_CHECK_HIP(hipGetLastError());
  return VK_OK;
}

template <typename T, int CIN, int TC, bool UP, int MODE>
static int launch_stream(const HaloParams& p, hipStream_t st) {
  using Cfg = StreamCfg<T, CIN, UP>;
  HaloParams q = p;
  const char* e_rs = getenv("VK_STREAM_RS");
  int RS = Cfg::RS;
  if (e_rs) {
    RS = atoi(e_rs);
  } else {
    const long per_row_block = (long)p.N * ((p.W + 15) / 16);
    while (RS * 2 <= 256 && per_row_block * ((p.H + 2 * RS - 1) / (2 * RS)) >= 4096) RS *= 2;
  }
  RS = (RS + 7) & ~7;
  if (RS < 8) RS = 8;
  q.tiles_y = RS;
  const long strips = (long)p.N * ((p.H + RS - 1) / RS) * ((p.W + 15) / 16);
  dim3 grid((unsigned)((strips + 3) / 4), 1, 1);
  static const std::string tag_f = std::string("stream_16b_c") + std::to_string(CIN) + (UP ? "up" : "") + "_k" + std::to_string(TC * 16);
  static const std::string tag_d = tag_f + "_dgrad";
  const std::string& tag = p.flip ? tag_d : tag_f;
  const double in_px = (double)p.N * (p.H >> (UP ? 1 : 0)) * (p.W >> (UP ? 1 : 0));
  const double out_px = (double)p.N * p.H * p.W * (p.pool2 ? 0.25 : 1.0);
  const double bytes = (in_px * CIN + out_px * p.K * (p.bnr_z ? 2.0 : 1.0) + 9.0 * p.K * CIN) * 2.0;
  vkh::ProfScope ps(tag.c_str(), st, 2.0 * (double)p.N * p.H * p.W * p.K * 9.0 * CIN, bytes);
  hipLaunchKernelGGL((conv3x3_stream_kernel<T, CIN, TC, UP, MODE>), grid, dim3(256), Cfg::SMEM, st, q);
  VK_CHECK_HIP(hipGetLastError());
  return VK_OK;
}

template <typename T>
static int stream_try(const HaloParams& p, hipStream_t st) {
  if (getenv("VK_NO_STREAM")) return VK_ERR_UNSUPPORTED;
  if (p.s1.ptr || p.accumulate || p.split || p.ld0 != p.K) return VK_ERR_UNSUPPORTED;
  const bool up = p.s0.up != 0, bnr = p.bnr_z != nullptr, pool = p.pool2 != 0;
  if ((pool || up) && ((p.H | p.W) & 1)) return VK_ERR_UNSUPPORTED;
  const bool fwd = !p.flip && !bnr && !pool;
  if (fwd && p.C == 32 && up && p.K == 16) return launch_stream<T, 32, 1, true, 0>(p, st);
  if (fwd && p.C == 16 && !up && p.K == 16) return launch_stream<T, 16, 1, false, 0>(p, st);
  if (fwd && p.C == 32 && !up && p.K == 32) return launch_stream<T, 32, 2, false, 0>(p, st);
  if (p.flip && !p.s0.scale && bnr && !pool && p.C == 16 && p.K == 16) return launch_stream<T, 16, 1, false, 2>(p, st);
  if (p.flip && !p.s0.scale && bnr && !pool && p.C == 32 && p.K == 32) return launch_stream<T, 32, 2, false, 2>(p, st);
  if (p.flip && !p.s0.scale && bnr && pool && p.C == 16 && p.K == 32) return launch_stream<T, 16, 2, false, 3>(p, st);
  return VK_ERR_UNSUPPORTED;
}

int conv3x3_halo_try(const vk_conv_desc* d, const void* w, int packed, void* y, void* y1, int split_k1, int accumulate, double* stats,
                     int pool2, const vk_bnr* bnr, hipStream_t st, void* workspace, size_t workspace_bytes) {
  const bool s2 = d->stride == 2 && !d->transposed && d->H == 2 * d->Ho && d->W == 2 * d->Wo && d->K >= 128 && !d->src0.up && !d->src1.ptr &&
                  !pool2 && !bnr && !accumulate && !split_k1 && !getenv("VK_NO_S2_TILE");
  const bool s2d = d->stride == 2 && d->transposed && d->Ho == 2 * d->H && d->Wo == 2 * d->W && d->K >= 64 && d->K % 64 == 0 && !d->src0.up &&
                   !d->src1.ptr && !d->src0.scale && !pool2 && !bnr && !split_k1 && !getenv("VK_NO_S2_TILE");
  if (d->R != 3 || d->S != 3 || d->pad != 1) return VK_ERR_UNSUPPORTED;
  if (!s2 && !s2d && (d->stride != 1 || d->H != d->Ho || d->W != d->Wo)) return VK_ERR_UNSUPPORTED;
  const int eb = d->dtype == VK_F32 ? 4 : 2;
  const int ck = 64 / eb;
  const int C = d->src0.C + (d->src1.ptr ? d->src1.C : 0);
  const bool c16 = (eb == 2) && C == 16 && !d->src1.ptr && !d->src0.up && !s2 && !s2d;
  if (c16 ? packed : !packed) return VK_ERR_UNSUPPORTED;
  if (!c16 && (d->src0.C % ck || (d->src1.ptr && d->src1.C % ck))) return VK_ERR_UNSUPPORTED;
  if (d->K % 16) return VK_ERR_UNSUPPORTED;
  if (pool2 && ((d->H | d->W) & 1)) return VK_ERR_UNSUPPORTED;
  if (d->src1.ptr && d->src1.up) return VK_ERR_UNSUPPORTED;
  if ((size_t)d->N * d->H * d->W * C * eb >= (1ull << 31) || (size_t)d->N * d->H * d->W >= (1ull << 31)) return VK_ERR_UNSUPPORTED;
  if (s2d && (size_t)d->N * d->Ho * d->Wo * d->K * eb >= (1ull << 32)) return VK_ERR_UNSUPPORTED;
  HaloParams p;
  auto mk = [&](const vk_src& s) {
    HaloSrc h;
    h.ptr = s.ptr; h.scale = s.scale; h.shift = s.shift; h.C = s.C; h.up = s.up; h.relu = s.relu;
    h.bytes = s.ptr ? (uint32_t)((size_t)d->N * (d->H >> s.up) * (d->W >> s.up) * s.C * eb) : 0u;
    return h;
  };
  p.s0 = mk(d->src0);
  if (d->src1.ptr) p.s1 = mk(d->src1);
  else p.s1 = HaloSrc{nullptr, nullptr, nullptr, 0, 0, 0, 0u};
  p.w = w;
  p.w_bytes = (uint32_t)((size_t)d->K * 9 * C * eb);
  p.y0 = y; p.y1 = y1; p.split = split_k1;
  p.ld0 = split_k1 ? split_k1 : d->K;
  p.ld1 = split_k1 ? d->K - split_k1 : 0;
  p.stats = stats;
  p.N = d->N; p.H = d->Ho; p.W = d->Wo; p.K = d->K; p.C = C;
  p.Hi = d->H; p.Wi = d->W;
  p.flip = d->transposed;
  p.accumulate = accumulate;
  p.pool2 = pool2;
  p.ksplit = 1;
  p.kyn = 0;
  p.slab = (reinterpret_cast<uintptr_t>(workspace) & 15) ? nullptr : (float*)workspace;
  p.slab_bytes = p.slab ? workspace_bytes : 0;
  p.stamps = nullptr;
  p.dbg = getenv("VK_COL_DBG") ? atoi(getenv("VK_COL_DBG")) : 0;
  if (p.dbg & 1) p.w_bytes = 0;
#ifdef VK_STAMP
  { extern unsigned long long* g_vk_stamp_buf; p.stamps = g_vk_stamp_buf; }
#endif
  p.bnr_z = bnr ? bnr->z : nullptr;
  p.bnr_scale = bnr ? bnr->scale : nullptr;
  p.bnr_shift = bnr ? bnr->shift : nullptr;
  p.bnr_sums = bnr ? bnr->sums : nullptr;
  p.bnr_mask = bnr ? bnr->mask : nullptr;
  p.nchunks = c16 ? 1 : C / ck;
  if (p.bnr_mask && (c16 || s2 || s2d || pool2)) return VK_ERR_UNSUPPORTED;
  if (eb == 2 && !s2 && !s2d && !p.bnr_mask && (c16 || C == 32)) {
    const int rc = d->dtype == VK_BF16 ? stream_try<bf16_t>(p, st) : stream_try<f16_t>(p, st);
    if (rc != VK_ERR_UNSUPPORTED) return rc;
  }
  if (c16) {
    if (d->dtype == VK_BF16) return d->K >= 32 ? launch_c16<bf16_t, 32>(p, st) : launch_c16<bf16_t, 16>(p, st);
    return d->K >= 32 ? launch_c16<f16_t, 32>(p, st) : launch_c16<f16_t, 16>(p, st);
  }
  p.tiles_x = p.tiles_y = 0;
  if (s2d) {
    p.flip = 0;
    const long tiles = (long)d->N * ((d->H + 7) / 8) * ((d->W + 15) / 16);
    const bool wide = d->K % 128 == 0 && tiles * (d->K / 128) >= 256;
    switch (d->dtype) {
      case VK_F32: return wide ? launch_s2dg<float, 128>(p, st) : launch_s2dg<float, 64>(p, st);
      case VK_BF16: return wide ? launch_s2dg<bf16_t, 128>(p, st) : launch_s2dg<bf16_t, 64>(p, st);
      case VK_F16: return wide ? launch_s2dg<f16_t, 128>(p, st) : launch_s2dg<f16_t, 64>(p, st);
    }
    return VK_ERR_ARG;
  }
  if (s2) {
    p.slab = nullptr;
    p.slab_bytes = 0;
    switch (d->dtype) {
      case VK_F32: return launch_col<float, 8, 128, 2, 4, false, 1, 0, 2>(p, st);
      case VK_BF16: return launch_col<bf16_t, 8, 128, 2, 4, false, 1, 0, 2>(p, st);
      case VK_F16: return launch_col<f16_t, 8, 128, 2, 4, false, 1, 0, 2>(p, st);
    }
    return VK_ERR_ARG;
  }
  switch (d->dtype) {
    case VK_F32: return halo_select<float>(p, st);
    case VK_BF16: return halo_select<bf16_t>(p, st);
    case VK_F16: return halo_select<f16_t>(p, st);
  }
  return VK_ERR_ARG;
}

}

extern "C" int vk_dec4_tail_eval(vk_dtype dtype, int N, int H, int W, const vk_src* src, const void* w1_pack, const float* scale1,
                                 const float* shift1, const void* w2_plain, const float* scale2, const float* shift2, const float* head_w9x16,
                                 const float* head_bias, float* logits, void* stream) {
  return vk::dec4_tail_eval_impl(dtype, N, H, W, src, w1_pack, scale1, shift1, w2_plain, scale2, shift2, head_w9x16, head_bias, logits,
                                 (hipStream_t)stream);
}
```

### vickers-hardness-unet_amd/csrc/engine.hip

```cpp
#include <stdarg.h>
#include <stdio.h>
#include <stdlib.h>
#include <string.h>

#include <algorithm>
#include <atomic>
#include <map>
#include <mutex>
#include <string>
#include <vector>

#include "vk_common.h"

namespace vkh {
static thread_local char g_err[512] = "";
void set_error(const char* fmt, ...) {
  va_list ap;
  va_start(ap, fmt);
  vsnprintf(g_err, sizeof(g_err), fmt, ap);
  va_end(ap);
}

struct ProfRec {
  std::string tag;
// ... 972 lines not shown
    e.src = c.w_off; e.dst = c.wd_off; e.K = c.K; e.RS = c.R * c.R; e.C = c.Cin; e.pad_ = 0;
    h->pack_tab.push_back(e);
  }
  h->cast_tab.clear();
  for (size_t i = 0; i < h->convs.size(); ++i) {
    const ConvL& c = h->convs[i];
    if ((int)i == h->stem_conv || (int)i == h->head_conv || c.halo_fwd) continue;
    h->cast_tab.push_back(CastRange{c.w_off, (int64_t)c.K * c.Cin * c.R * c.R});
  }
  h->bn_tab.clear();
  for (const BnL& b : h->bns) {
    BnEvalEntry e;
    e.g_off = b.g_off; e.b_off = b.b_off; e.rm_off = b.rm_off; e.rv_off = b.rv_off; e.out_off = b.arena_off; e.C = b.C; e.pad_ = 0;
    h->bn_tab.push_back(e);
  }
  if (!h->pack_tab.empty())
    VK_CHECK_HIP(hipMemcpy(h->ws + h->off_tab_pack, h->pack_tab.data(), h->pack_tab.size() * sizeof(PackEntry), hipMemcpyHostToDevice));
  if (!h->halo_tab.empty())
    VK_CHECK_HIP(hipMemcpy(h->ws + h->off_tab_halo, h->halo_tab.data(), h->halo_tab.size() * sizeof(HaloPackEntry), hipMemcpyHostToDevice));
  if (!h->cast_tab.empty())
    VK_CHECK_HIP(hipMemcpy(h->ws + h->off_tab_cast, h->cast_tab.data(), h->cast_tab.size() * sizeof(CastRange), hipMemcpyHostToDevice));
  VK_CHECK_HIP(hipMemcpy(h->ws + h->off_tab_bn, h->bn_tab.data(), h->bn_tab.size() * sizeof(BnEvalEntry), hipMemcpyHostToDevice));
  if (h->cfg.training && !h->side && getenv("VK_SIDE_STREAM")) RET_IF(vk_unet_set_side_stream(h, 1));
  h->bound = true;
  return VK_OK;
}

template <typename T>
static int refresh_t(vk_unet* h, hipStream_t st) {
  vkh::ProfScope ps_("weights_repack", st, 0.0, (double)h->n_params * (4.0 + 2.0 * sizeof(T)));
  if (sizeof(T) != 4 && !h->cast_tab.empty())
    hipLaunchKernelGGL(k_cast_ranges<T>, dim3(16, (unsigned)h->cast_tab.size()), dim3(256), 0, st, (const CastRange*)(h->ws + h->off_tab_cast),
                       h->params, (T*)(h->ws + h->off_wf));
  if (h->cfg.training && !h->pack_tab.empty())
    hipLaunchKernelGGL(k_pack_dgrad<T>, dim3(64, (unsigned)h->pack_tab.size()), dim3(256), 0, st,
                       (const PackEntry*)(h->ws + h->off_tab_pack), h->params, (T*)(h->ws + h->off_wd));
  if (!h->halo_tab.empty())
    hipLaunchKernelGGL(k_pack_halo_tab<T>, dim3(32, (unsigned)h->halo_tab.size()), dim3(256), 0, st,
                       (const HaloPackEntry*)(h->ws + h->off_tab_halo), h->params, h->ws);
  hipLaunchKernelGGL(k_pack_stem<T>, dim3((64 * 7 * 32 + 255) / 256), dim3(256), 0, st,
                     h->params + h->convs[h->stem_conv].w_off, (T*)(h->ws + h->off_wstem));
  VK_CHECK_HIP(hipGetLastError());
  return VK_OK;
}

extern "C" int vk_unet_refresh_weights(vk_unet* h, void* stream) {
  VK_CHECK_ARG(h && h->bound, "vk_unet_refresh_weights: plan not bound");
  hipStream_t st = (hipStream_t)stream;
  switch (h->cfg.dtype) {
    case VK_F32: return refresh_t<float>(h, st);
    case VK_BF16: return refresh_t<bf16_t>(h, st);
    case VK_F16: return refresh_t<f16_t>(h, st);
  }
  return VK_ERR_ARG;
}

extern "C" int vk_unet_set_side_stream(vk_unet* h, int enable) {
  VK_CHECK_ARG(h, "vk_unet_set_side_stream: null plan");
  if (enable && !h->side && h->cfg.training) {
    VK_CHECK_HIP(hipStreamCreateWithFlags(&h->side, hipStreamNonBlocking));
    VK_CHECK_HIP(hipEventCreateWithFlags(&h->ev_fork, hipEventDisableTiming));
    VK_CHECK_HIP(hipEventCreateWithFlags(&h->ev_join, hipEventDisableTiming));
  } else if (!enable && h->side) {
    VK_CHECK_HIP(hipStreamSynchronize(h->side));
    (void)hipEventDestroy(h->ev_fork);
    (void)hipEventDestroy(h->ev_join);
    (void)hipStreamDestroy(h->side);
    h->side = nullptr;
    h->ev_fork = h->ev_join = nullptr;
    h->side_dirty = false;
  }
  return VK_OK;
}

extern "C" int vk_unet_set_trainable(vk_unet* h, const uint8_t* flags, int n) {
  VK_CHECK_ARG(h && flags, "vk_unet_set_trainable: null argument");
  VK_CHECK_ARG(n == h->n_ptensors, "vk_unet_set_trainable: %d flags for %d parameter tensors", n, h->n_ptensors);
  bool changed = false;
  for (int t = 0; t < n; ++t) {
    const uint8_t v = flags[t] ? 1 : 0;
    changed |= v != h->trainable[(size_t)t];
    h->trainable[(size_t)t] = v;
  }
  if (!changed) return VK_OK;
  update_last_rank(h);
  ++h->mask_version;
  return VK_OK;
}

extern "C" int vk_unet_set_bn_frozen(vk_unet* h, const uint8_t* flags, int n) {
  VK_CHECK_ARG(h && flags, "vk_unet_set_bn_frozen: null argument");
  VK_CHECK_ARG(n == (int)h->bns.size(), "vk_unet_set_bn_frozen: %d flags for %d BatchNorm layers", n, (int)h->bns.size());
  static_assert(sizeof(h->bn_frozen) * 8 >= kMaxBnLayers, "one bit per BatchNorm layer");
  uint64_t m = 0;
  for (int l = 0; l < n; ++l) m |= (flags[l] ? 1ull : 0ull) << l;
  h->bn_frozen = m;
  return VK_OK;
}

extern "C" int vk_unet_set_input_grad(vk_unet* h, float* dx) {
  VK_CHECK_ARG(h, "vk_unet_set_input_grad: null plan");
  VK_CHECK_ARG(!dx || h->cfg.training, "vk_unet_set_input_grad: needs a training plan");
  h->dx_in = dx;
  update_last_rank(h);
  return VK_OK;
}

extern "C" int vk_unet_zero_grad(vk_unet* h, void* stream) {
  VK_CHECK_ARG(h && h->bound && h->grads, "vk_unet_zero_grad: no gradient buffer bound");
  VK_CHECK_HIP(hipMemsetAsync(h->grads, 0, (size_t)h->n_params * sizeof(float), (hipStream_t)stream));
  return VK_OK;
}

extern "C" int vk_unet_debug_tensor(const vk_unet* h, const char* name, void** ptr, int dims[4]) {
  VK_CHECK_ARG(h && h->bound && name && ptr && dims, "vk_unet_debug_tensor: bad argument");
  auto it = h->debug.find(name);
  VK_CHECK_ARG(it != h->debug.end(), "vk_unet_debug_tensor: unknown tensor '%s'", name);
  *ptr = it->second.first;
  for (int i = 0; i < 4; ++i) dims[i] = i < (int)it->second.second.size() ? it->second.second[i] : 1;
  return VK_OK;
}

extern "C" int vk_unet_forward(vk_unet* h, const float* x, float* logits, int training, void* stream) {
  VK_CHECK_ARG(h && h->bound && x && logits, "vk_unet_forward: plan not bound or null tensor");
  VK_CHECK_ARG(!training || h->cfg.training, "vk_unet_forward: training forward needs a training plan");
  hipStream_t st = (hipStream_t)stream;
  const int N = h->cfg.N, S = h->cfg.size, SW = h->cfg.width;
  const vk_dtype dt = h->cfg.dtype;
  if (training) {
    h->bn_frozen_fwd = h->bn_frozen;
    VK_CHECK_HIP(hipMemsetAsync(h->ws + h->off_stats, 0, h->stats_bytes, st));
    if (h->bn_frozen_fwd) {
      hipLaunchKernelGGL(k_bn_frozen_affine, dim3((unsigned)h->bns.size()), dim3(128), 0, st, (const BnEvalEntry*)(h->ws + h->off_tab_bn),
                         h->bn_frozen_fwd, h->params, h->bufs, (float*)(h->ws + h->off_farena), 1e-5f);
      VK_CHECK_HIP(hipGetLastError());
    }
  } else {
    hipLaunchKernelGGL(k_bn_eval_all, dim3((unsigned)h->bns.size()), dim3(128), 0, st, (const BnEvalEntry*)(h->ws + h->off_tab_bn),
                       h->params, h->bufs, (float*)(h->ws + h->off_farena), 1e-5f);
    VK_CHECK_HIP(hipGetLastError());
  }
  void* x4 = h->ws + h->off_x4;
  RET_IF(vk_input_transform(dt, N, S, SW, x, x4, st));
  ConvL& stem = h->convs[h->stem_conv];
  BnL& sbn = h->bns[stem.bn];
  RET_IF(vk_stem_fwd(dt, N, S, SW, x4, h->ws + h->off_wstem, stem.z, training && !frozen(h, sbn) ? sbn.stats : nullptr, st));
  RET_IF(finalize_bn(h, sbn, training, st));
  void* pool = h->ws + h->off_pool;
  RET_IF(vk_bn_relu_maxpool(dt, N, S / 2, SW / 2, 64, stem.z, sbn.scale, sbn.shift, pool, (uint8_t*)(h->ws + h->off_argmax), st));
  Act cur{pool, 64, nullptr, nullptr, 0};
  for (BlockL& k : h->blocks) {
    ConvL& c1 = h->convs[k.conv1];
    ConvL& c2 = h->convs[k.conv2];
    RET_IF(run_conv(h, c1, to_src(cur), null_src(), training, st));
    RET_IF(run_conv(h, c2, to_src(bn_act(h, c1)), null_src(), training, st));
    ConvL& ct = k.conv3 >= 0 ? h->convs[k.conv3] : c2;
    if (k.conv3 >= 0) RET_IF(run_conv(h, ct, to_src(bn_act(h, c2)), null_src(), training, st));
    const BnL& b2 = h->bns[ct.bn];
    const size_t pixels = (size_t)N * k.Hout * k.Wout;
    if (k.convd >= 0) {
      ConvL& cd = h->convs[k.convd];
      RET_IF(run_conv(h, cd, to_src(cur), null_src(), training, st));
      const BnL& bd = h->bns[cd.bn];
      RET_IF(vk_bn_add_relu(dt, pixels, k.C, ct.z, b2.scale, b2.shift, cd.z, bd.scale, bd.shift, k.out, st));
    } else {
      RET_IF(vk_bn_add_relu(dt, pixels, k.C, ct.z, b2.scale, b2.shift, cur.ptr, nullptr, nullptr, k.out, st));
    }
    cur = Act{k.out, k.C, nullptr, nullptr, 0};
  }
  Act skips[5];
  for (int i = 0; i < 3; ++i) {
    const BlockL& fb = h->blocks[h->layer_last_block[2 - i]];
    skips[i] = Act{fb.out, fb.C, nullptr, nullptr, 0};
  }
  skips[3] = bn_act(h, stem);
  skips[4] = Act{nullptr, 0, nullptr, nullptr, 0};
  Act xd = cur;
  for (size_t i = 0; i < h->decs.size(); ++i) {
    DecL& d = h->decs[i];
    ConvL& c1 = h->convs[d.conv1];
    ConvL& c2 = h->convs[d.conv2];
    const bool small_plan = (size_t)N * S * SW <= 4u * 512 * 512;
    if (!training && h->classes == 1 && i + 1 == h->decs.size() && dt != VK_F32 && !d.Cskip && d.Cup == 32 && c1.K == 16 && c2.K == 16 && c1.halo_fwd &&
        !c2.halo_fwd && S % 16 == 0 && SW % 16 == 0 && !getenv("VK_NO_TAIL_FUSION") && (small_plan || getenv("VK_TAIL_FUSION"))) {
      const vk_src s0 = to_src(xd, 1);
      const BnL& b1 = h->bns[c1.bn];
      const BnL& b2 = h->bns[c2.bn];
      return vk_dec4_tail_eval(dt, N, S, SW, &s0, fwd_weights(h, c1), b1.scale, b1.shift, fwd_weights(h, c2), b2.scale, b2.shift,
                               h->params + h->head_w_off, h->params + h->head_b_off, logits, st);
    }
    RET_IF(run_conv(h, c1, to_src(xd, 1), d.Cskip ? to_src(skips[i]) : null_src(), training, st));
    RET_IF(run_conv(h, c2, to_src(bn_act(h, c1)), null_src(), training, st));
    xd = bn_act(h, c2);
  }
  vk_src hs = to_src(xd);
  if (h->classes == 1) RET_IF(vk_head_fwd(dt, N, S, SW, &hs, h->params + h->head_w_off, h->params + h->head_b_off, logits, st));
  else RET_IF(vk_head_fwd_multi(dt, N, S, SW, h->classes, &hs, h->params + h->head_w_off, h->params + h->head_b_off, logits, st));
  if (training) {
    if (h->bn_frozen_fwd) hipLaunchKernelGGL(k_inc_i64_masked, dim3(1), dim3(64), 0, st, (int)h->bns.size(), h->nbt, h->bn_frozen_fwd);
    else hipLaunchKernelGGL(k_inc_i64, dim3(1), dim3(64), 0, st, (int)h->bns.size(), h->nbt);
    VK_CHECK_HIP(hipGetLastError());
  }
  return VK_OK;
}

extern "C" int vk_unet_loss_ex(vk_unet* h, int mode, const void* logits, const void* target, float* loss_out, float grad_scale,
                               float w_ce, float w_dice, void* stream) {
  VK_CHECK_ARG(h && h->bound && logits && target && loss_out, "vk_unet_loss_ex: plan not bound or null tensor");
  VK_CHECK_ARG(mode == VK_LOSS_BINARY || mode == VK_LOSS_MULTILABEL || mode == VK_LOSS_MULTICLASS, "vk_unet_loss_ex: bad mode %d", mode);
  VK_CHECK_ARG(mode != VK_LOSS_BINARY || h->classes == 1, "vk_unet_loss_ex: the binary loss needs classes == 1 (the plan has %d)", h->classes);
  VK_CHECK_ARG(mode != VK_LOSS_MULTICLASS || h->classes >= 2, "vk_unet_loss_ex: the multi-class loss needs classes >= 2");
  if (h->classes == 1) return vk_unet_loss(h, (const float*)logits, (const float*)target, loss_out, grad_scale, w_ce, w_dice, stream);
  const int N = h->cfg.N, HW = h->cfg.size * h->cfg.width;
  float* dl = h->cfg.training ? (float*)(h->ws + h->off_dlogits) : nullptr;
  if (mode == VK_LOSS_MULTILABEL)
    return vk_multilabel_loss(N, h->classes, HW, (const float*)logits, (const float*)target, h->ws + h->off_mloss, h->mloss_bytes, loss_out,
                              dl, grad_scale, w_ce, w_dice, stream);
  return vk_multiclass_loss(N, h->classes, HW, (const float*)logits, (const int64_t*)target, h->ws + h->off_mloss, h->mloss_bytes, loss_out,
                            dl, grad_scale, w_ce, w_dice, stream);
}

extern "C" int vk_unet_loss_cfg(vk_unet* h, const vk_seg_loss_cfg* cfg, const void* logits, const void* target, float* loss_out,
                                float grad_scale, void* stream) {
  VK_CHECK_ARG(h && h->bound && cfg && logits && target && loss_out, "vk_unet_loss_cfg: plan not bound or null argument");
  float* dl = h->cfg.training ? (float*)(h->ws + h->off_dlogits) : nullptr;
  return vk_seg_loss(cfg, h->cfg.N, h->classes, h->cfg.size * h->cfg.width, (const float*)logits, target, h->ws + h->off_sloss,
                     h->sloss_bytes, loss_out, dl, grad_scale, stream);
}

extern "C" int vk_unet_loss_lovasz(vk_unet* h, const vk_seg_loss_cfg* seg_cfg, const vk_lovasz_cfg* lovasz_cfg, float w_lovasz,
                                   const void* logits, const void* target, void* workspace, size_t workspace_bytes, float* loss_out,
                                   float grad_scale, void* stream) {
  VK_CHECK_ARG(h && h->bound && lovasz_cfg && logits && target && workspace && loss_out,
               "vk_unet_loss_lovasz: plan not bound or null argument");
  VK_CHECK_ARG(w_lovasz == w_lovasz && w_lovasz - w_lovasz == 0.f, "vk_unet_loss_lovasz: w_lovasz is not finite");
  VK_CHECK_ARG(!seg_cfg || seg_cfg->mode == lovasz_cfg->mode, "vk_unet_loss_lovasz: the two parts disagree on the mode");
  const int N = h->cfg.N, HW = h->cfg.size * h->cfg.width;
  float* dl = h->cfg.training ? (float*)(h->ws + h->off_dlogits) : nullptr;
  hipStream_t st = (hipStream_t)stream;
  if (seg_cfg) RET_IF(vk_seg_loss(seg_cfg, N, h->classes, HW, (const float*)logits, target, h->ws + h->off_sloss, h->sloss_bytes, loss_out,
                                  dl, grad_scale, stream));
  else VK_CHECK_HIP(hipMemsetAsync(loss_out, 0, 8 * sizeof(float), st));
  RET_IF(vk_lovasz_loss(lovasz_cfg, N, h->classes, HW, (const float*)logits, target, workspace, workspace_bytes, loss_out + 8, dl,
                        grad_scale * w_lovasz, seg_cfg ? 1 : 0, stream));
  return vk::lovasz_combine(loss_out, w_lovasz, st);
}

extern "C" int vk_unet_loss(vk_unet* h, const float* logits, const float* target, float* loss_out, float grad_scale, float w_bce,
                            float w_dice, void* stream) {
  VK_CHECK_ARG(h && h->bound && logits && target && loss_out, "vk_unet_loss: plan not bound or null tensor");
  VK_CHECK_ARG(h->classes == 1, "vk_unet_loss: the binary loss needs classes == 1; use vk_unet_loss_ex");
  const size_t count = (size_t)h->cfg.N * h->cfg.size * h->cfg.width;
  float* dl = h->cfg.training ? (float*)(h->ws + h->off_dlogits) : nullptr;
  return vk_bce_dice_loss(count, logits, target, (double*)(h->ws + h->off_loss_sums), loss_out, dl, grad_scale, w_bce, w_dice, stream);
}

#ifndef VK_BN_APPLY_FUSED_MAXC_DEFAULT
#define VK_BN_APPLY_FUSED_MAXC_DEFAULT 0
#endif
namespace {

int bn_bwd_phase2(vk_unet* h, BnL& b, int C, size_t pixels, const void* dy, const void* z, int mask_mode, const void* mask_src, void* dz,
                  void* g_out, int g_acc, hipStream_t st) {
  static const int maxc = getenv("VK_BN_APPLY_FUSED_MAXC") ? atoi(getenv("VK_BN_APPLY_FUSED_MAXC")) : VK_BN_APPLY_FUSED_MAXC_DEFAULT;
  if (frozen(h, b)) {
    if (trains(h, b.g_t) || trains(h, b.b_t))
      RET_IF(vk_bn_bwd_coeffs_frozen(C, b.bsums, h->params + b.g_off, b.mean, b.invstd, dgamma_of(h, b), dbeta_of(h, b), b.coef, st));
    return vk_bn_bwd_apply(h->cfg.dtype, pixels, C, dy, z, mask_mode, b.scale, b.shift, mask_src, b.coef, dz, g_out, g_acc, st);
  }
  if (C <= maxc)
    return vk_bn_bwd_apply_fused(h->cfg.dtype, pixels, C, dy, z, mask_mode, b.scale, b.shift, mask_src, b.bsums, b.count, h->params + b.g_off,
                                 b.mean, b.invstd, dgamma_of(h, b), dbeta_of(h, b), dz, g_out, g_acc, st);
  RET_IF(vk_bn_bwd_coeffs(C, b.bsums, b.count, h->params + b.g_off, b.mean, b.invstd, dgamma_of(h, b), dbeta_of(h, b), b.coef, st));
  return vk_bn_bwd_apply(h->cfg.dtype, pixels, C, dy, z, mask_mode, b.scale, b.shift, mask_src, b.coef, dz, g_out, g_acc, st);
}

int bn_relu_bwd_inplace(vk_unet* h, ConvL& c, bool prereduced, hipStream_t st) {
  BnL& b = h->bns[c.bn];
  const size_t pixels = (size_t)h->cfg.N * c.Hout * c.Wout;
  if (!prereduced && bn_sums_needed(h, b)) RET_IF(vk_bn_bwd_reduce(h->cfg.dtype, pixels, c.K, c.g, c.z, 1, b.scale, b.shift, nullptr, b.bsums, st));
  return bn_bwd_phase2(h, b, c.K, pixels, c.g, c.z, prereduced ? 0 : 1, nullptr, c.g, nullptr, 0, st);
}

int wgrad_stream(vk_unet* h, hipStream_t st, hipStream_t* out) {
  *out = st;
  if (!h->side) return VK_OK;
  VK_CHECK_HIP(hipEventRecord(h->ev_fork, st));
  VK_CHECK_HIP(hipStreamWaitEvent(h->side, h->ev_fork, 0));
  h->side_dirty = true;
  *out = h->side;
  return VK_OK;
}

int join_side(vk_unet* h, hipStream_t st) {
  if (!h->side || !h->side_dirty) return VK_OK;
  VK_CHECK_HIP(hipEventRecord(h->ev_join, h->side));
  VK_CHECK_HIP(hipStreamWaitEvent(st, h->ev_join, 0));
  h->side_dirty = false;
  return VK_OK;
}

int conv_wgrad(vk_unet* h, ConvL& c, const vk_src& s0, const vk_src& s1, hipStream_t st) {
  vk_conv_desc d = conv_desc(h, c, s0, s1);
  if (!h->side && vk::wgrad_batch_supports(&d)) {
    h->pending.push_back(vk_unet::WItem{d, c.g, h->grads + c.w_off});
    return VK_OK;
  }
  hipStream_t ws;
  RET_IF(wgrad_stream(h, st, &ws));
  return vk_conv_wgrad(&d, c.g, h->grads + c.w_off, h->ws + h->off_wslab, VK_WGRAD_WORKSPACE_BYTES, ws);
}

vk_bnr bnr_of(vk_unet* h, ConvL& target) {
  BnL& b = h->bns[target.bn];
  vk_bnr r;
// ... 45 lines not shown
  const int rc = vk_conv_bwd_onepass(&d, c.g, c.z, b.coef, dgrad_weights(h, c), into.g, &r, h->grads + c.w_off, h->ws + h->off_wslab,
                                     VK_WGRAD_WORKSPACE_BYTES, st);
  if (rc == VK_ERR_UNSUPPORTED) {
    *state = 2;
    return vk_bn_bwd_apply(h->cfg.dtype, (size_t)h->cfg.N * c.Hout * c.Wout, c.K, c.g, c.z, 0, b.scale, b.shift, nullptr, b.coef, c.g, nullptr, 0, st);
  }
  *state = rc == VK_OK ? 1 : 0;
  return rc;
}

int conv_dgrad(vk_unet* h, ConvL& c, void* y, void* y1, int split, int accumulate, hipStream_t st) {
  vk_conv_desc d;
  d.dtype = h->cfg.dtype;
  d.N = h->cfg.N; d.H = c.Hout; d.W = c.Wout; d.Ho = c.Hin; d.Wo = c.Win;
  d.K = c.Cin; d.R = c.R; d.S = c.R; d.stride = c.stride; d.pad = c.pad; d.transposed = 1;
  vk_src s;
  s.ptr = c.g; s.C = c.K; s.up = 0; s.scale = nullptr; s.shift = nullptr; s.relu = 0;
  d.src0 = s;
  d.src1 = null_src();
  if (on_1x1(c) && !split) return vk_conv1x1_fwd(&d, dgrad_weights(h, c), y, accumulate, nullptr, st);
  if (c.halo_dg) return vk_conv_fwd_packed(&d, dgrad_weights(h, c), y, y1, split, accumulate, nullptr, st);
  return vk_conv_fwd(&d, dgrad_weights(h, c), y, y1, split, accumulate, nullptr, st);
}

int backward_decoder(vk_unet* h, int i, hipStream_t st) {
  DecL& d = h->decs[i];
  ConvL& c1 = h->convs[d.conv1];
  ConvL& c2 = h->convs[d.conv2];
  const int N = h->cfg.N;
  ConvL& stem = h->convs[h->stem_conv];
  Act xprev, skip{nullptr, 0, nullptr, nullptr, 0};
  void* g_prev;
  if (i == 0) {
    BlockL& f5 = h->blocks[h->layer_last_block[3]];
    xprev = Act{f5.out, f5.C, nullptr, nullptr, 0};
    g_prev = f5.gout;
  } else {
    ConvL& pc2 = h->convs[h->decs[i - 1].conv2];
    xprev = bn_act(h, pc2);
    g_prev = pc2.g;
  }
  void* g_skip = nullptr;
  if (i <= 2) {
    BlockL& fb = h->blocks[h->layer_last_block[2 - i]];
    skip = Act{fb.out, fb.C, nullptr, nullptr, 0};
    g_skip = fb.gout;
  } else if (i == 3) {
    skip = bn_act(h, stem);
    g_skip = stem.g;
  }
  const BnL& bn1 = h->bns[c1.bn];
  if (!need_from(h, h->bns[c2.bn].rank)) {
    if (i > 0) h->g_prereduced[h->decs[i - 1].conv2] = 0;
    return VK_OK;
  }
  const bool into1 = need_from(h, bn1.rank);
  bool fused1 = false;
  int onepass = 0;
  if (h->g_prereduced[d.conv2] && into1 && trains(h, c2.w_t) && h->cfg.dtype != VK_F32 && !h->side && !on_1x1(c2) && !getenv("VK_NO_ONEPASS") &&
      !getenv("VK_NO_BNR_FUSION"))
    RET_IF(conv_bwd_onepass(h, c2, c1, 0, &onepass, st));
  if (onepass == 1) {
    fused1 = true;
  } else {
    if (onepass == 0) RET_IF(bn_relu_bwd_inplace(h, c2, h->g_prereduced[d.conv2] != 0, st));
    if (into1) RET_IF(conv_dgrad_into(h, c2, c1, &fused1, st));
    if (trains(h, c2.w_t)) RET_IF(conv_wgrad(h, c2, to_src(bn_act(h, c1)), null_src(), st));
  }
  if (i > 0) h->g_prereduced[h->decs[i - 1].conv2] = 0;
  if (!into1) return VK_OK;
  int onepass1 = 0;
  if (fused1 && i > 0 && !d.Cskip && trains(h, c1.w_t) && need_from(h, c1.rank + 1) && h->cfg.dtype != VK_F32 && !h->side && !on_1x1(c1) &&
      !getenv("VK_NO_ONEPASS") && !getenv("VK_NO_ONEPASS_UP") && !getenv("VK_NO_BNR_FUSION"))
    RET_IF(conv_bwd_onepass(h, c1, h->convs[h->decs[i - 1].conv2], 1, &onepass1, st));
  if (onepass1 == 1) {
    h->g_prereduced[h->decs[i - 1].conv2] = 1;
    return VK_OK;
  }
  if (onepass1 == 0) RET_IF(bn_relu_bwd_inplace(h, c1, fused1, st));
  if (need_from(h, c1.rank + 1)) {
    vk_conv_desc dd = dgrad_desc(h, c1);
    vk_bnr r;
    const bool want_bnr = i > 0 && !getenv("VK_NO_BNR_FUSION");
    if (want_bnr) r = bnr_of(h, h->convs[h->decs[i - 1].conv2]);
    const int rc = vk_conv_dgrad_fused(&dd, dgrad_weights(h, c1), g_prev, d.Cskip ? g_skip : nullptr, d.Cskip ? d.Cup : 0, 1,
                                       want_bnr ? &r : nullptr, st);
    if (rc == VK_OK && want_bnr) h->g_prereduced[h->decs[i - 1].conv2] = 1;
    if (rc != VK_OK && rc != VK_ERR_UNSUPPORTED) return rc;
    if (rc == VK_ERR_UNSUPPORTED) {
      void* dup = h->ws + h->off_dup;
      if (d.Cskip) RET_IF(conv_dgrad(h, c1, dup, g_skip, d.Cup, 0, st));
      else RET_IF(conv_dgrad(h, c1, dup, nullptr, 0, 0, st));
      RET_IF(vk_upsample2x_bwd(h->cfg.dtype, N, d.H, d.W, d.Cup, dup, g_prev, 0, st));
    }
  }
  if (!trains(h, c1.w_t)) return VK_OK;
  return conv_wgrad(h, c1, to_src(xprev, 1), d.Cskip ? to_src(skip) : null_src(), st);
}

int backward_block(vk_unet* h, int bi, hipStream_t st) {
  BlockL& k = h->blocks[bi];
  ConvL& c1 = h->convs[k.conv1];
  ConvL& c2 = h->convs[k.conv2];
  BnL& b2 = h->bns[c2.bn];
  const vk_dtype dt = h->cfg.dtype;
  const size_t pixels = (size_t)h->cfg.N * k.Hout * k.Wout;
  if (!need_from(h, b2.rank)) {
    h->tail_prereduced[(size_t)bi] = 0;
    return VK_OK;
  }
  Act xin;
  void* gin;
  if (bi == 0) {
    xin = Act{h->ws + h->off_pool, 64, nullptr, nullptr, 0};
    gin = h->ws + h->off_gpool;
  } else {
    BlockL& pb = h->blocks[bi - 1];
    xin = Act{pb.out, pb.C, nullptr, nullptr, 0};
    gin = pb.gout;
  }
  const bool pre = h->tail_prereduced[(size_t)bi] != 0;
  h->tail_prereduced[(size_t)bi] = 0;
  if (bi > 0) h->tail_prereduced[(size_t)bi - 1] = 0;
  const int mm = pre ? 0 : 2;
  if (!pre && bn_sums_needed(h, b2)) RET_IF(vk_bn_bwd_reduce(dt, pixels, k.C, k.gout, c2.z, 2, nullptr, nullptr, k.out, b2.bsums, st));
  if (k.convd < 0) {
    RET_IF(bn_bwd_phase2(h, b2, k.C, pixels, k.gout, c2.z, mm, k.out, c2.g, gin, k.in_has_grad_first ? 1 : 0, st));
  } else {
    ConvL& cd = h->convs[k.convd];
    BnL& bd = h->bns[cd.bn];
    RET_IF(bn_bwd_phase2(h, b2, k.C, pixels, k.gout, c2.z, mm, k.out, c2.g, nullptr, 0, st));
    if (bn_sums_needed(h, bd)) RET_IF(vk_bn_bwd_reduce(dt, pixels, k.C, k.gout, cd.z, mm, nullptr, nullptr, k.out, bd.bsums, st));
    RET_IF(bn_bwd_phase2(h, bd, k.C, pixels, k.gout, cd.z, mm, k.out, cd.g, nullptr, 0, st));
  }
  const bool into1 = need_from(h, h->bns[c1.bn].rank);
  bool fused1 = false;
  if (into1) RET_IF(conv_dgrad_into(h, c2, c1, &fused1, st));
  if (trains(h, c2.w_t)) RET_IF(conv_wgrad(h, c2, to_src(bn_act(h, c1)), null_src(), st));
  if (!into1) return k.convd >= 0 && trains(h, h->convs[k.convd].w_t) ? conv_wgrad(h, h->convs[k.convd], to_src(xin), null_src(), st) : VK_OK;
  RET_IF(bn_relu_bwd_inplace(h, c1, fused1, st));
  const bool into_gin = need_from(h, c1.rank + 1);
  bool tail_fused = false;
  const int tail_maxc = getenv("VK_TAIL_BNR_MAXC") ? atoi(getenv("VK_TAIL_BNR_MAXC")) : 1 << 20;
  if (into_gin && k.convd < 0 && bi > 0 && c1.halo_dg && k.C <= tail_maxc && !getenv("VK_NO_TAIL_BNR_FUSION")) {
    BlockL& pb = h->blocks[bi - 1];
    ConvL& pc2 = h->convs[pb.conv2];
    vk_conv_desc dd = dgrad_desc(h, c1);
    vk_bnr r;
    r.z = pc2.z; r.scale = nullptr; r.shift = nullptr; r.sums = h->bns[pc2.bn].bsums; r.mask = pb.out; r.accumulate = 1;
    const int rc = vk_conv_dgrad_fused(&dd, dgrad_weights(h, c1), gin, nullptr, 0, 0, &r, st);
    if (rc == VK_OK) { tail_fused = true; h->tail_prereduced[(size_t)bi - 1] = 1; }
    else if (rc != VK_ERR_UNSUPPORTED) return rc;
  }
  if (into_gin && !tail_fused) RET_IF(conv_dgrad(h, c1, gin, nullptr, 0, 1, st));
  if (k.convd >= 0) {
    ConvL& cd = h->convs[k.convd];
    if (into_gin) RET_IF(conv_dgrad(h, cd, gin, nullptr, 0, 1, st));
    if (trains(h, c1.w_t)) RET_IF(conv_wgrad(h, c1, to_src(xin), null_src(), st));
    return trains(h, cd.w_t) ? conv_wgrad(h, cd, to_src(xin), null_src(), st) : VK_OK;
  }
  return trains(h, c1.w_t) ? conv_wgrad(h, c1, to_src(xin), null_src(), st) : VK_OK;
}

int backward_bottleneck(vk_unet* h, int bi, hipStream_t st) {
  BlockL& k = h->blocks[bi];
  ConvL& c1 = h->convs[k.conv1];
  ConvL& c2 = h->convs[k.conv2];
  ConvL& c3 = h->convs[k.conv3];
  BnL& b3 = h->bns[c3.bn];
  const vk_dtype dt = h->cfg.dtype;
  const size_t pixels = (size_t)h->cfg.N * k.Hout * k.Wout;
  h->tail_prereduced[(size_t)bi] = 0;
  if (!need_from(h, b3.rank)) return VK_OK;
  Act xin;
  void* gin;
  if (bi == 0) {
    xin = Act{h->ws + h->off_pool, 64, nullptr, nullptr, 0};
    gin = h->ws + h->off_gpool;
  } else {
    BlockL& pb = h->blocks[bi - 1];
    xin = Act{pb.out, pb.C, nullptr, nullptr, 0};
    gin = pb.gout;
  }
  bool gin_written = k.in_has_grad_first;
  if (bn_sums_needed(h, b3)) RET_IF(vk_bn_bwd_reduce(dt, pixels, k.C, k.gout, c3.z, 2, nullptr, nullptr, k.out, b3.bsums, st));
  if (k.convd < 0) {
    RET_IF(bn_bwd_phase2(h, b3, k.C, pixels, k.gout, c3.z, 2, k.out, c3.g, gin, gin_written ? 1 : 0, st));
    gin_written = true;
  } else {
    RET_IF(bn_bwd_phase2(h, b3, k.C, pixels, k.gout, c3.z, 2, k.out, c3.g, nullptr, 0, st));
    ConvL& cd = h->convs[k.convd];
    BnL& bd = h->bns[cd.bn];
    if (need_from(h, bd.rank)) {
      if (bn_sums_needed(h, bd)) RET_IF(vk_bn_bwd_reduce(dt, pixels, k.C, k.gout, cd.z, 2, nullptr, nullptr, k.out, bd.bsums, st));
      RET_IF(bn_bwd_phase2(h, bd, k.C, pixels, k.gout, cd.z, 2, k.out, cd.g, nullptr, 0, st));
    }
  }
  const bool into2 = need_from(h, h->bns[c2.bn].rank);
  if (into2) RET_IF(conv_dgrad(h, c3, c2.g, nullptr, 0, 0, st));
  if (trains(h, c3.w_t)) RET_IF(conv_wgrad(h, c3, to_src(bn_act(h, c2)), null_src(), st));
  if (k.convd >= 0 && trains(h, h->convs[k.convd].w_t)) RET_IF(conv_wgrad(h, h->convs[k.convd], to_src(xin), null_src(), st));
  if (!into2) return VK_OK;
  RET_IF(bn_relu_bwd_inplace(h, c2, false, st));
  const bool into1 = need_from(h, h->bns[c1.bn].rank);
  bool fused1 = false;
  if (into1) RET_IF(conv_dgrad_into(h, c2, c1, &fused1, st));
  if (trains(h, c2.w_t)) RET_IF(conv_wgrad(h, c2, to_src(bn_act(h, c1)), null_src(), st));
  if (!into1) return VK_OK;
  RET_IF(bn_relu_bwd_inplace(h, c1, fused1, st));
  if (need_from(h, c1.rank + 1)) {
    RET_IF(conv_dgrad(h, c1, gin, nullptr, 0, gin_written ? 1 : 0, st));
    if (k.convd >= 0) RET_IF(conv_dgrad(h, h->convs[k.convd], gin, nullptr, 0, 1, st));
  }
  return trains(h, c1.w_t) ? conv_wgrad(h, c1, to_src(xin), null_src(), st) : VK_OK;
}

int stem_coeffs(vk_unet* h, BnL& b, hipStream_t st) {
  if (!frozen(h, b))
    return vk_bn_bwd_coeffs(64, b.bsums, b.count, h->params + b.g_off, b.mean, b.invstd, dgamma_of(h, b), dbeta_of(h, b), b.coef, st);
  if (!trains(h, b.g_t) && !trains(h, b.b_t)) return VK_OK;
  return vk_bn_bwd_coeffs_frozen(64, b.bsums, h->params + b.g_off, b.mean, b.invstd, dgamma_of(h, b), dbeta_of(h, b), b.coef, st);
}

int backward_stem(vk_unet* h, hipStream_t st) {
  const int N = h->cfg.N, S = h->cfg.size, SW = h->cfg.width;
  ConvL& stem = h->convs[h->stem_conv];
  if (!need_from(h, h->bns[stem.bn].rank)) return VK_OK;
  BnL& b = h->bns[stem.bn];
  const bool want_w = trains(h, stem.w_t);
  const float* const w = h->params + stem.w_off;
  if (getenv("VK_NO_POOL_BNR_FUSION")) {
    RET_IF(vk_maxpool_bwd(h->cfg.dtype, N, S / 2, SW / 2, 64, h->ws + h->off_gpool, (const uint8_t*)(h->ws + h->off_argmax), stem.g, st));
    RET_IF(bn_relu_bwd_inplace(h, stem, false, st));
  } else {
    RET_IF(vk_maxpool_bwd_bn_reduce(h->cfg.dtype, N, S / 2, SW / 2, 64, h->ws + h->off_gpool, (const uint8_t*)(h->ws + h->off_argmax), stem.z,
                                    b.scale, b.shift, stem.g, b.bsums, st));
    if (!want_w && !h->dx_in) return stem_coeffs(h, b, st);
    if (h->cfg.dtype != VK_F32 && !getenv("VK_NO_STEM_BNA")) {
      RET_IF(stem_coeffs(h, b, st));
      int rc = VK_OK;
      if (want_w) {
        hipStream_t ws;
        RET_IF(wgrad_stream(h, st, &ws));
        rc = vk_stem_wgrad_bn(h->cfg.dtype, N, S, SW, h->ws + h->off_x4, stem.g, stem.z, b.coef, h->grads + stem.w_off,
                              h->ws + h->off_wslab, VK_WGRAD_WORKSPACE_BYTES, ws);
        if (rc != VK_OK && rc != VK_ERR_UNSUPPORTED) return rc;
      }
      if (rc == VK_OK) return h->dx_in ? vk_stem_dgrad(h->cfg.dtype, N, S, SW, stem.g, stem.z, b.coef, w, h->dx_in, st) : VK_OK;
      RET_IF(vk_bn_bwd_apply(h->cfg.dtype, (size_t)N * (S / 2) * (SW / 2), 64, stem.g, stem.z, 0, b.scale, b.shift, nullptr, b.coef, stem.g, nullptr, 0, st));
    } else {
      RET_IF(bn_relu_bwd_inplace(h, stem, true, st));
    }
  }
  if (want_w) {
    hipStream_t ws;
    RET_IF(wgrad_stream(h, st, &ws));
    RET_IF(vk_stem_wgrad(h->cfg.dtype, N, S, SW, h->ws + h->off_x4, stem.g, h->grads + stem.w_off, h->ws + h->off_wslab, VK_WGRAD_WORKSPACE_BYTES, ws));
  }
  return h->dx_in ? vk_stem_dgrad(h->cfg.dtype, N, S, SW, stem.g, nullptr, nullptr, w, h->dx_in, st) : VK_OK;
}

int flush_wgrads(vk_unet* h, int stage, hipStream_t st) {
  const int n = (int)h->pending.size();
  if (n == 0) return VK_OK;
  char* const slab = h->ws + h->off_wslab;
  auto each = [&]() {
    int rc = VK_OK;
    for (const vk_unet::WItem& it : h->pending) {
      rc = vk_conv_wgrad(&it.d, it.dz, it.dw, slab, kEngineSlabBytes, st);
      if (rc != VK_OK) break;
    }
    h->pending.clear();
    return rc;
  };
  if (n == 1 || n > kMaxBatch || stage < 0 || stage >= kMaxStages) return each();
  const int target = 256 - vkh::reserved_cus();
  const int slot = target == 256 ? 0 : 1;
  vk_unet::WPlan& wp = h->wplans[stage][slot];
  char* const tables = h->ws + h->off_tab_wbatch + ((size_t)stage * 2 + slot) * VK_WGRAD_BATCH_TABLE_BYTES;
  if (!wp.built || wp.target != target || wp.n != n || wp.version != h->mask_version) {
    if (wp.built) VK_CHECK_HIP(hipStreamSynchronize(st));
    vk_conv_desc descs[kMaxBatch];
    const void* dz[kMaxBatch];
    float* dw[kMaxBatch];
    for (int i = 0; i < n; ++i) { descs[i] = h->pending[(size_t)i].d; dz[i] = h->pending[(size_t)i].dz; dw[i] = h->pending[(size_t)i].dw; }
    wp.plan = vk::WgradBatchPlan();
    const int rc = vk::wgrad_batch_build(descs, dz, dw, n, target, tables, VK_WGRAD_BATCH_TABLE_BYTES, &wp.plan);
    if (rc != VK_OK) { h->pending.clear(); return rc; }
    wp.built = true; wp.target = target; wp.n = n; wp.version = h->mask_version;
  }
  if (wp.plan.slab_need > kEngineSlabBytes) return each();
  const int rc = vk::wgrad_batch_launch(h->cfg.dtype, wp.plan, tables, slab, kEngineSlabBytes, st);
  h->pending.clear();
  return rc;
}

int backward_stage(vk_unet* h, const float* dlogits, int stage, hipStream_t st) {
  const int N = h->cfg.N, S = h->cfg.size, SW = h->cfg.width;
  switch (stage) {
    case 0: {
      if (!need_from(h, 0)) return VK_OK;
      VK_CHECK_HIP(hipMemsetAsync(h->ws + h->off_bsums, 0, h->stats_bytes, st));
      ConvL& last = h->convs[h->decs[4].conv2];
      const ConvL& head = h->convs[h->head_conv];
      float* const hdw = grad_or_sink(h, head.w_t, h->head_w_off, 2 * h->sink_c);
      float* const hdb = grad_or_sink(h, head.b_t, h->head_b_off, 2 * h->sink_c + 144 * h->classes);
      vk_src hs = to_src(bn_act(h, last));
      if (h->classes > 1) {
        vk_bnr r = bnr_of(h, last);
        const float* dl = dlogits ? dlogits : (const float*)(h->ws + h->off_dlogits);
// ... 46 lines not shown
```

Before: 3033.

## Fuse stride-2 1x1 downsample shortcut into the 3x3 conv forward and dgrad kernels

Adds a shortcut variant (SC template flag) to the stride-2 column conv kernel, so the 1x1 stride-2 downsample conv runs in the same pass. It reuses the centre-tap input fragments already in registers and writes a second output with its own BN stats. The stride-2 dgrad kernel gets the same treatment: the shortcut's transposed 1x1 contribution accumulates into the parity-0 output, and the optional BN-ReLU tail fusion is kept. This removes separate kernel launches and a re-read of the block input in BasicBlock downsampling stages. In exchange it costs extra accumulators, more LDS for the shortcut weights and dz, and a second epilogue pass.

```diff
diff --git a/include/vk_unet.h b/include/vk_unet.h
--- a/include/vk_unet.h
+++ b/include/vk_unet.h
@@ -61,6 +61,9 @@
 #define VK_SPLITK_WORKSPACE_BYTES (32u << 20)
 int vk_conv_fwd_splitk(const vk_conv_desc* d, const void* w_halo, void* y, void* workspace, size_t workspace_bytes, void* stream);
 
+int vk_conv_fwd_s2sc(const vk_conv_desc* d, const void* w_halo, const vk_conv_desc* d_sc, const void* w_sc, void* z, void* z_sc,
+                     double* stats, double* stats_sc, void* stream);
+
 typedef struct {
   const void* z;
   const float* scale;
@@ -72,6 +75,9 @@
 
 int vk_conv_dgrad_fused(const vk_conv_desc* d, const void* w, void* y, void* y1, int split_k1, int pool2, const vk_bnr* bnr,
                         void* stream);
+
+int vk_conv_dgrad_s2sc(const vk_conv_desc* d, const void* w_halo, const vk_conv_desc* d_sc, const void* w_sc, void* y, int accumulate,
+                       const vk_bnr* bnr, void* stream);
 
 int vk_conv1x1_fwd(const vk_conv_desc* d, const void* w, void* y, int accumulate, double* stats, void* stream);
 int vk_conv1x1_wgrad(const vk_conv_desc* d, const void* dz, float* dw, void* workspace, size_t workspace_bytes, void* stream);
diff --git a/vickers-hardness-unet_amd/_lib.py b/vickers-hardness-unet_amd/_lib.py
--- a/vickers-hardness-unet_amd/_lib.py
+++ b/vickers-hardness-unet_amd/_lib.py
@@ -124,6 +124,8 @@
     "vk_conv_uses_halo_pack": (ci, [P(vk_conv_desc)]),
     "vk_conv_fwd_packed": (ci, [P(vk_conv_desc), vp, vp, vp, ci, ci, vp, vp]),
     "vk_conv_fwd_splitk": (ci, [P(vk_conv_desc), vp, vp, vp, sz, vp]),
+    "vk_conv_fwd_s2sc": (ci, [P(vk_conv_desc), vp, P(vk_conv_desc), vp, vp, vp, vp, vp, vp]),
+    "vk_conv_dgrad_s2sc": (ci, [P(vk_conv_desc), vp, P(vk_conv_desc), vp, vp, ci, P(vk_bnr), vp]),
     "vk_stem_fwd": (ci, [ci, ci, ci, ci, vp, vp, vp, vp, vp]),
     "vk_conv_wgrad": (ci, [P(vk_conv_desc), vp, vp, vp, sz, vp]),
     "vk_conv1x1_fwd": (ci, [P(vk_conv_desc), vp, vp, ci, vp, vp]),
diff --git a/vickers-hardness-unet_amd/csrc/conv_halo.hip b/vickers-hardness-unet_amd/csrc/conv_halo.hip
--- a/vickers-hardness-unet_amd/csrc/conv_halo.hip
+++ b/vickers-hardness-unet_amd/csrc/conv_halo.hip
@@ -59,6 +59,12 @@
   const float* bnr_shift;
   double* bnr_sums;
   const void* bnr_mask;
+  const void* w2 = nullptr;
+  uint32_t w2_bytes = 0;
+  void* z2 = nullptr;
+  double* stats2 = nullptr;
+  const void* x2 = nullptr;
+  uint32_t x2_bytes = 0;
 };
 
 template <typename T, int TH, int BN, int WGM, int WGN>
@@ -538,7 +544,7 @@
 #endif
 }
 
-template <typename T, int TH, int BN, int WGM, int WGN, bool ADB, int STR = 1>
+template <typename T, int TH, int BN, int WGM, int WGN, bool ADB, int STR = 1, bool SC = false>
 struct ColCfg {
   using Tr = ElemTraits<T>;
   static constexpr int EB = Tr::kBytes;
@@ -560,19 +566,21 @@
   static constexpr int NX = STR * (TP - 1) + 3;
   static constexpr int ESB = BN * EB + 16;
   static constexpr int NB = (BN <= 64 && STR == 1) ? 3 : 2;
-  static constexpr int MAIN = NA * A_BYTES + NB * B_BYTES;
+  static constexpr int S_BYTES = SC ? BN * 64 : 0;
+  static constexpr int MAIN = NA * A_BYTES + NB * B_BYTES + S_BYTES;
   static constexpr int ESLOTS = (BN / VE > 16) ? NW * 4 / (BN / VE / 16) : NW * 4;
   static constexpr int EPI = BM * ESB + ESLOTS * BN * 2 * 4;
   static constexpr int SMEM = MAIN > EPI ? MAIN : EPI;
   static_assert(TH % WGM == 0 && BN % (16 * WGN) == 0 && (NW == 4 || NW == 8), "wave layout");
   static_assert(STR == 1 || STR == 2, "stride");
+  static_assert(!SC || (STR == 2 && !ADB && EB == 2), "the fused shortcut belongs to the 16-bit stride-2 tile");
   static_assert(SMEM <= 160 * 1024, "main-loop / epilogue LDS image exceeds the 160 KiB of a CU");
   static_assert(EPI >= BM * ESB + ESLOTS * BN * 8, "epilogue partial-sum slots must fit behind the output tile");
 };
 
-template <typename T, int TH, int BN, int WGM, int WGN, bool ADB, int MINW, int STR = 1>
+template <typename T, int TH, int BN, int WGM, int WGN, bool ADB, int MINW, int STR = 1, bool SC = false>
 __global__ __launch_bounds__(64 * WGM * WGN, MINW) void conv3x3_col_kernel(const HaloParams p) {
-  using Cfg = ColCfg<T, TH, BN, WGM, WGN, ADB, STR>;
+  using Cfg = ColCfg<T, TH, BN, WGM, WGN, ADB, STR, SC>;
   constexpr int EB = Cfg::EB, VE = Cfg::VE, CK = Cfg::CK, HPIX = Cfg::HPIX, NPV = Cfg::NPV, NT = Cfg::NT, NW = Cfg::NW;
   constexpr int TP = Cfg::TP, TC = Cfg::TC, APS = Cfg::APS, NPIECE = Cfg::NPIECE, RS = Cfg::RS, HWI = Cfg::HWI, NX = Cfg::NX;
   typedef __attribute__((address_space(3))) void lds_void;
@@ -684,6 +692,20 @@
     }
   };
 
+  char* const Sbuf = Bbuf + Cfg::NB * Cfg::B_BYTES;
+  const __amdgpu_buffer_rsrc_t rsw2 = make_rsrc(SC ? p.w2 : p.w, SC ? p.w2_bytes : 0u);
+  const uint32_t sc_voff = (uint32_t)((lane >> 2) * p.C * EB) + (uint32_t)(((lane & 3) ^ swz(lane >> 2)) << 4);
+  auto dma_sc = [&](int cc) {
+#pragma unroll
+    for (int i = 0; i < (BN / 16 + NW - 1) / NW; ++i) {
+      const int pc = wave + i * NW;
+      if ((BN / 16) % NW == 0 || pc < BN / 16) {
+        const uint32_t goff = (uint32_t)((n0 + pc * 16) * p.C + cc * CK) * (uint32_t)EB;
+        __builtin_amdgcn_raw_ptr_buffer_load_lds(rsw2, (lds_void*)(Sbuf + pc * (16 * 64)), 16, sc_voff, goff, 0, 0);
+      }
+    }
+  };
+
   const int wrow0 = (wave / WGN) * TP;
   const int wch0 = (wave % WGN) * (TC * 16);
   f32x4_t acc[TC][TP];
@@ -691,11 +713,17 @@
   for (int a = 0; a < TC; ++a)
 #pragma unroll
     for (int b = 0; b < TP; ++b) acc[a][b] = f32x4_t{0.f, 0.f, 0.f, 0.f};
+  f32x4_t acc2[SC ? TC : 1][SC ? TP : 1];
+#pragma unroll
+  for (int a = 0; a < (SC ? TC : 1); ++a)
+#pragma unroll
+    for (int b = 0; b < (SC ? TP : 1); ++b) acc2[a][b] = f32x4_t{0.f, 0.f, 0.f, 0.f};
   const int li = lane & 15, kg = lane >> 4;
   const int a_lane = (STR * wrow0 * RS + li) * APS + kg * 16;
   const int b_lane = (wch0 + li) * 64 + ((kg ^ swz(li)) << 4);
 
-  auto compute = [&](const char* A, const char* B) {
+  auto compute = [&](const char* A, const char* B, auto cen_c) {
+    constexpr bool CEN = decltype(cen_c)::value;
     u32x4_t X[NX], W[3][TC];
 #pragma unroll
     for (int h = 0; h < NX; ++h) X[h] = *reinterpret_cast<const u32x4_t*>(A + h * (RS * APS));
@@ -709,13 +737,24 @@
       for (int a = 0; a < TC; ++a)
 #pragma unroll
         for (int b = 0; b < TP; ++b) acc[a][b] = Mma<T>::run(W[r][a], X[STR * b + r], acc[a][b]);
+    if constexpr (CEN) {
+      u32x4_t W2[TC];
+#pragma unroll
+      for (int a = 0; a < TC; ++a) W2[a] = *reinterpret_cast<const u32x4_t*>(Sbuf + b_lane + (a * 16) * 64);
+#pragma unroll
+      for (int a = 0; a < TC; ++a)
+#pragma unroll
+        for (int b = 0; b < TP; ++b) acc2[a][b] = Mma<T>::run(W2[a], X[STR * b + 1], acc2[a][b]);
+    }
     constexpr int NM = TC * TP * (sizeof(T) == 4 ? 4 : 1);
     __builtin_amdgcn_sched_group_barrier(0x100, NX + TC, 0);
     __builtin_amdgcn_sched_group_barrier(0x100, TC, 0);
     __builtin_amdgcn_sched_group_barrier(0x008, NM, 0);
     __builtin_amdgcn_sched_group_barrier(0x100, TC, 0);
     __builtin_amdgcn_sched_group_barrier(0x008, NM, 0);
+    if constexpr (CEN) __builtin_amdgcn_sched_group_barrier(0x100, TC, 0);
     __builtin_amdgcn_sched_group_barrier(0x008, NM, 0);
+    if constexpr (CEN) __builtin_amdgcn_sched_group_barrier(0x008, NM, 0);
   };
 
 #ifdef VK_STAMP
@@ -739,7 +778,8 @@
   if (one_chunk) {
     const char* A = Abuf + a_lane;
 #pragma unroll
-    for (int s = 0; s < 3; ++s) compute(A + (STR == 1 ? s : (s & 1) * 17 + (s >> 1)) * APS, Bbuf + s * Cfg::B_BYTES + b_lane);
+    for (int s = 0; s < 3; ++s)
+      compute(A + (STR == 1 ? s : (s & 1) * 17 + (s >> 1)) * APS, Bbuf + s * Cfg::B_BYTES + b_lane, std::false_type{});
     __syncthreads();
     st = 3;
   }
@@ -757,9 +797,17 @@
         if (s < 2) dma_b(cc, s + 1, (st + 1) & 1);
         else if (next_chunk) dma_b(cc + 1, 0, (st + 1) & 1);
       }
+      if (SC && s == 0) dma_sc(cc);
       if (s == 0 && next_chunk && !(p.dbg & 4)) load_halo(cc + 1);
       VK_T(t1)
-      compute(A + (STR == 1 ? s : (s & 1) * 17 + (s >> 1)) * APS, Bbuf + (st & 1) * Cfg::B_BYTES + b_lane);
+      const char* const As = A + (STR == 1 ? s : (s & 1) * 17 + (s >> 1)) * APS;
+      const char* const Bs = Bbuf + (st & 1) * Cfg::B_BYTES + b_lane;
+      if constexpr (SC) {
+        if (s == 1) compute(As, Bs, std::true_type{});
+        else compute(As, Bs, std::false_type{});
+      } else {
+        compute(As, Bs, std::false_type{});
+      }
       VK_T(t2)
       if (ADB) {
         if (s == 1 && next_chunk && !(p.dbg & 4)) store_halo(Anext);
@@ -793,6 +841,13 @@
     return;
   }
   halo_epilogue<T, TH, BN, TP, TC, NT, (BN <= 64 && TH == 16)>(smem, acc, p, n, y0, x0, n0, wrow0, wch0);
+  if constexpr (SC) {
+    __syncthreads();
+    HaloParams q = p;
+    q.y0 = p.z2;
+    q.stats = p.stats2;
+    halo_epilogue<T, TH, BN, TP, TC, NT, false>(smem, acc2, q, n, y0, x0, n0, wrow0, wch0);
+  }
 #ifdef VK_STAMP
   VK_T(te1)
   if (p.stamps && lane == 0) {
@@ -802,7 +857,7 @@
 #endif
 }
 
-template <typename T, int TH, int BN, int WGM, int WGN>
+template <typename T, int TH, int BN, int WGM, int WGN, bool SC = false>
 struct S2dCfg {
   using Tr = ElemTraits<T>;
   static constexpr int EB = Tr::kBytes, VE = Tr::kVec, CK = 64 / EB;
@@ -815,18 +870,21 @@
   static constexpr int BM = TH * 16;
   static constexpr int TP = TH / WGM, TC = BN / WGN / 16;
   static constexpr int ESB = BN * EB + 16;
-  static constexpr int MAIN = 2 * A_BYTES + 2 * B_BYTES;
+  static constexpr int SW_BYTES = SC ? BN * 64 : 0;
+  static constexpr int SX_BYTES = SC ? BM * 64 : 0;
+  static constexpr int MAIN = 2 * A_BYTES + 2 * B_BYTES + SW_BYTES + SX_BYTES;
   static constexpr int ESLOTS = (BN / VE > 16) ? NW * 4 / (BN / VE / 16) : NW * 4;
   static constexpr int EPI = BM * ESB + ESLOTS * BN * 2 * 4;
   static constexpr int SMEM = MAIN > EPI ? MAIN : EPI;
+  static_assert(!SC || EB == 2, "the fused shortcut belongs to the 16-bit plans");
   static_assert(TH % WGM == 0 && BN % (16 * WGN) == 0 && NW == 8, "wave layout");
   static_assert(4 * TP * TC <= 32, "accumulator budget (four parity classes)");
   static_assert(SMEM <= 160 * 1024, "LDS image exceeds the 160 KiB of a CU");
 };
 
-template <typename T, int TH, int BN, int WGM, int WGN>
+template <typename T, int TH, int BN, int WGM, int WGN, bool SC = false>
 __global__ __launch_bounds__(64 * WGM * WGN, 1) void conv3x3_s2dg_kernel(const HaloParams p) {
-  using Cfg = S2dCfg<T, TH, BN, WGM, WGN>;
+  using Cfg = S2dCfg<T, TH, BN, WGM, WGN, SC>;
   constexpr int EB = Cfg::EB, VE = Cfg::VE, CK = Cfg::CK, HPIX = Cfg::HPIX, NPV = Cfg::NPV, NT = Cfg::NT, NW = Cfg::NW;
   constexpr int TP = Cfg::TP, TC = Cfg::TC, APS = Cfg::APS, NPIECE = Cfg::NPIECE, RS = Cfg::RS;
   typedef __attribute__((address_space(3))) void lds_void;
@@ -892,6 +950,31 @@
     }
   };
 
+  char* const Swbuf = Bbuf + 2 * Cfg::B_BYTES;
+  char* const Sxbuf = Swbuf + Cfg::SW_BYTES;
+  const __amdgpu_buffer_rsrc_t rsw2 = make_rsrc(SC ? p.w2 : p.w, SC ? p.w2_bytes : 0u);
+  const __amdgpu_buffer_rsrc_t rsx2 = make_rsrc(SC ? p.x2 : p.s0.ptr, SC ? p.x2_bytes : 0u);
+  const uint32_t sc_piece = (uint32_t)(((lane & 3) ^ swz(lane >> 2)) << 4);
+  const uint32_t sc_wvoff = (uint32_t)((lane >> 2) * p.C * EB) + sc_piece;
+  static_assert(!SC || TH <= NW, "one tile row of the shortcut's dz per wave");
+  uint32_t sc_xvoff = kOOB;
+  {
+    const int y = y0 + wave, x = x0 + (lane >> 2);
+    if (SC && wave < TH && y < p.Hi && x < p.Wi) sc_xvoff = (uint32_t)(((n * p.Hi + y) * p.Wi + x) * p.C * EB) + sc_piece;
+  }
+  auto dma_sc = [&](int cc) {
+#pragma unroll
+    for (int i = 0; i < (BN / 16 + NW - 1) / NW; ++i) {
+      const int pc = wave + i * NW;
+      if ((BN / 16) % NW == 0 || pc < BN / 16) {
+        const uint32_t goff = (uint32_t)((n0 + pc * 16) * p.C + cc * CK) * (uint32_t)EB;
+        __builtin_amdgcn_raw_ptr_buffer_load_lds(rsw2, (lds_void*)(Swbuf + pc * (16 * 64)), 16, sc_wvoff, goff, 0, 0);
+      }
+    }
+    if (TH == NW || wave < TH)
+      __builtin_amdgcn_raw_ptr_buffer_load_lds(rsx2, (lds_void*)(Sxbuf + wave * (16 * 64)), 16, sc_xvoff, (uint32_t)(cc * 64), 0, 0);
+  };
+
   const int wrow0 = (wave / WGN) * TP;
   const int wch0 = (wave % WGN) * (TC * 16);
   f32x4_t acc[4][TC][TP];
@@ -905,6 +988,8 @@
   const int a_lane = (wrow0 * RS + li) * APS + kg * 16;
   const int b_lane = (wch0 + li) * 64 + ((kg ^ swz(li)) << 4);
 
+  const int x2_lane = (wrow0 * 16 + li) * 64 + ((kg ^ swz(li)) << 4);
+
   auto compute = [&](const char* A, const char* B, auto s_c) {
     constexpr int s = decltype(s_c)::value;
     u32x4_t X[TP + 1], W[3][TC];
@@ -922,6 +1007,17 @@
       for (int a = 0; a < TC; ++a)
 #pragma unroll
         for (int b = 0; b < TP; ++b) acc[q][a][b] = Mma<T>::run(W[r][a], X[b + di], acc[q][a][b]);
+    }
+    if constexpr (SC && s == 1) {
+      u32x4_t W2[TC], X2[TP];
+#pragma unroll
+      for (int a = 0; a < TC; ++a) W2[a] = *reinterpret_cast<const u32x4_t*>(Swbuf + b_lane + (a * 16) * 64);
+#pragma unroll
+      for (int b = 0; b < TP; ++b) X2[b] = *reinterpret_cast<const u32x4_t*>(Sxbuf + x2_lane + b * (16 * 64));
+#pragma unroll
+      for (int a = 0; a < TC; ++a)
+#pragma unroll
+        for (int b = 0; b < TP; ++b) acc[0][a][b] = Mma<T>::run(W2[a], X2[b], acc[0][a][b]);
     }
   };
 
@@ -935,6 +1031,7 @@
     const char* A = Abuf + (cc & 1) * Cfg::A_BYTES + a_lane;
     char* const Anext = Abuf + ((cc + 1) & 1) * Cfg::A_BYTES;
     dma_b(cc, 1, (st + 1) & 1);
+    if (SC) dma_sc(cc);
     if (next_chunk) load_halo(cc + 1);
     compute(A, Bbuf + (st & 1) * Cfg::B_BYTES + b_lane, std::integral_constant<int, 0>{});
     __syncthreads();
@@ -2630,23 +2727,24 @@
   return VK_OK;
 }
 
-template <typename T, int BN>
+template <typename T, int BN, bool SC = false>
 static int launch_s2dg(HaloParams p, hipStream_t st) {
-  using Cfg = S2dCfg<T, 8, BN, 4, 2>;
+  using Cfg = S2dCfg<T, 8, BN, 4, 2, SC>;
   p.tiles_x = (p.Wi + 15) / 16;
   p.tiles_y = (p.Hi + 7) / 8;
   dim3 grid((unsigned)(p.N * p.tiles_y * p.tiles_x), (unsigned)((p.K + BN - 1) / BN), 1);
   static bool attr_done = false;
   if (!attr_done && Cfg::SMEM > 64 * 1024) {
-    VK_CHECK_HIP(hipFuncSetAttribute((const void*)conv3x3_s2dg_kernel<T, 8, BN, 4, 2>, hipFuncAttributeMaxDynamicSharedMemorySize, Cfg::SMEM));
+    VK_CHECK_HIP(hipFuncSetAttribute((const void*)conv3x3_s2dg_kernel<T, 8, BN, 4, 2, SC>, hipFuncAttributeMaxDynamicSharedMemorySize, Cfg::SMEM));
     attr_done = true;
   }
   {
-    static const std::string tag = std::string("s2dg_") + (sizeof(T) == 4 ? "f32" : "16b") + "_bn" + std::to_string(BN);
+    static const std::string tag = std::string("s2dg_") + (sizeof(T) == 4 ? "f32" : "16b") + "_bn" + std::to_string(BN) + (SC ? "_sc" : "");
     const std::string dtag = getenv("VK_PROF_DETAIL") ? tag + ":H" + std::to_string(p.H) + "_K" + std::to_string(p.K) + "_C" + std::to_string(p.C) : tag;
-    const double bytes = ((double)p.N * ((double)p.Hi * p.Wi * p.C + (double)p.H * p.W * p.K * (p.accumulate ? 2.0 : 1.0)) + 9.0 * p.K * p.C) * sizeof(T);
-    vkh::ProfScope ps(dtag.c_str(), st, 2.0 * (double)p.N * p.Hi * p.Wi * p.K * 9.0 * p.C, bytes);
-    hipLaunchKernelGGL((conv3x3_s2dg_kernel<T, 8, BN, 4, 2>), grid, dim3(Cfg::NT), Cfg::SMEM, st, p);
+    const double taps = SC ? 10.0 : 9.0;
+    const double bytes = ((double)p.N * ((double)p.Hi * p.Wi * p.C * (SC ? 2.0 : 1.0) + (double)p.H * p.W * p.K * (p.accumulate ? 2.0 : 1.0)) + taps * p.K * p.C) * sizeof(T);
+    vkh::ProfScope ps(dtag.c_str(), st, 2.0 * (double)p.N * p.Hi * p.Wi * p.K * taps * p.C, bytes);
+    hipLaunchKernelGGL((conv3x3_s2dg_kernel<T, 8, BN, 4, 2, SC>), grid, dim3(Cfg::NT), Cfg::SMEM, st, p);
   }
   VK_CHECK_HIP(hipGetLastError());
   return VK_OK;
@@ -2792,6 +2890,141 @@
   return VK_ERR_ARG;
 }
 
+template <typename T>
+static int launch_s2sc(HaloParams p, hipStream_t st) {
+  using Cfg = ColCfg<T, 8, 128, 2, 4, false, 2, true>;
+  const void* const kernel = (const void*)conv3x3_col_kernel<T, 8, 128, 2, 4, false, 1, 2, true>;
+  p.tiles_x = (p.W + 15) / 16;
+  p.tiles_y = (p.H + 7) / 8;
+  dim3 grid((unsigned)(p.N * p.tiles_y * p.tiles_x), (unsigned)(p.K / 128), 1);
+  p.ksplit = 1;
+  p.kyn = 0;
+  if (grid.y > 1 && (grid.x & 7) == 0 && !getenv("VK_COL_NO_KYFAST")) {
+    p.kyn = (int)grid.y;
+    grid.x *= grid.y;
+    grid.y = 1;
+  }
+  static bool attr_done = false;
+  if (!attr_done) {
+    VK_CHECK_HIP(hipFuncSetAttribute(kernel, hipFuncAttributeMaxDynamicSharedMemorySize, Cfg::SMEM));
+    attr_done = true;
+  }
+  {
+    static const std::string tag = "col_16b_t8_bn128_w8_s2sc";
+    const std::string dtag = getenv("VK_PROF_DETAIL") ? tag + ":H" + std::to_string(p.H) + "_K" + std::to_string(p.K) + "_C" + std::to_string(p.C) : tag;
+    const double macs = (double)p.N * p.H * p.W * p.K * 10.0 * p.C;
+    const double bytes = ((double)p.N * ((double)p.Hi * p.Wi * p.C + 2.0 * p.H * p.W * p.K) + 10.0 * p.K * p.C) * sizeof(T);
+    vkh::ProfScope ps(dtag.c_str(), st, 2.0 * macs, bytes);
+    void* args[] = {(void*)&p};
+    VK_CHECK_HIP(hipLaunchKernel(kernel, grid, dim3(Cfg::NT), args, Cfg::SMEM, st));
+  }
+  VK_CHECK_HIP(hipGetLastError());
+  return VK_OK;
+}
+
+int conv3x3_s2sc_impl(const vk_conv_desc* d, const void* w_halo, const vk_conv_desc* dsc, const void* w_sc, void* z, void* zd, double* stats,
+                      double* stats_d, hipStream_t st) {
+  if (d->dtype != VK_BF16 && d->dtype != VK_F16) return VK_ERR_UNSUPPORTED;
+  if (dsc->dtype != d->dtype || d->transposed || dsc->transposed) return VK_ERR_UNSUPPORTED;
+  if (d->R != 3 || d->S != 3 || d->pad != 1 || d->stride != 2) return VK_ERR_UNSUPPORTED;
+  if (dsc->R != 1 || dsc->S != 1 || dsc->pad != 0 || dsc->stride != 2) return VK_ERR_UNSUPPORTED;
+  if (d->H != 2 * d->Ho || d->W != 2 * d->Wo || d->Ho < 1 || d->Wo < 1) return VK_ERR_UNSUPPORTED;
+  if (dsc->N != d->N || dsc->H != d->H || dsc->W != d->W || dsc->Ho != d->Ho || dsc->Wo != d->Wo || dsc->K != d->K) return VK_ERR_UNSUPPORTED;
+  const vk_src &a = d->src0, &b = dsc->src0;
+  if (d->src1.ptr || dsc->src1.ptr || a.up || b.up) return VK_ERR_UNSUPPORTED;
+  if (a.ptr != b.ptr || a.C != b.C || a.scale != b.scale || a.shift != b.shift || (a.scale && a.relu != b.relu)) return VK_ERR_UNSUPPORTED;
+  const int C = a.C;
+  if (d->K < 128 || d->K % 128 || C < 32 || C % 32) return VK_ERR_UNSUPPORTED;
+  if ((size_t)d->N * d->H * d->W * C * 2 >= (1ull << 31) || (size_t)d->K * C * 2 * 9 >= (1ull << 31)) return VK_ERR_UNSUPPORTED;
+  if (getenv("VK_NO_S2_TILE")) return VK_ERR_UNSUPPORTED;
+  HaloParams p;
+  p.s0 = HaloSrc{a.ptr, a.scale, a.shift, a.C, 0, a.relu, (uint32_t)((size_t)d->N * d->H * d->W * C * 2)};
+  p.s1 = HaloSrc{nullptr, nullptr, nullptr, 0, 0, 0, 0u};
+  p.w = w_halo;
+  p.w_bytes = (uint32_t)((size_t)d->K * 9 * C * 2);
+  p.y0 = z; p.y1 = nullptr; p.split = 0;
+  p.ld0 = d->K; p.ld1 = 0;
+  p.stats = stats;
+  p.N = d->N; p.H = d->Ho; p.W = d->Wo; p.K = d->K; p.C = C;
+  p.Hi = d->H; p.Wi = d->W;
+  p.flip = 0; p.accumulate = 0; p.pool2 = 0;
+  p.tiles_x = p.tiles_y = 0;
+  p.nchunks = C / 32;
+  p.stamps = nullptr;
+  p.kyn = 0; p.ksplit = 1;
+  p.slab_bytes = 0; p.slab = nullptr;
+  p.dbg = 0;
+  p.bnr_z = nullptr; p.bnr_scale = nullptr; p.bnr_shift = nullptr; p.bnr_sums = nullptr; p.bnr_mask = nullptr;
+  p.w2 = w_sc;
+  p.w2_bytes = (uint32_t)((size_t)d->K * C * 2);
+  p.z2 = zd;
+  p.stats2 = stats_d;
+  return d->dtype == VK_BF16 ? launch_s2sc<bf16_t>(p, st) : launch_s2sc<f16_t>(p, st);
+}
+
+int conv3x3_s2sc_dgrad_impl(const vk_conv_desc* d, const void* w_halo, const vk_conv_desc* dsc, const void* w_sc, void* y, int accumulate,
+                            const vk_bnr* bnr, hipStream_t st) {
+  if (d->dtype != VK_BF16 && d->dtype != VK_F16) return VK_ERR_UNSUPPORTED;
+  if (dsc->dtype != d->dtype || !d->transposed || !dsc->transposed) return VK_ERR_UNSUPPORTED;
+  if (d->R != 3 || d->S != 3 || d->pad != 1 || d->stride != 2) return VK_ERR_UNSUPPORTED;
+  if (dsc->R != 1 || dsc->S != 1 || dsc->pad != 0 || dsc->stride != 2) return VK_ERR_UNSUPPORTED;
+  if (d->Ho != 2 * d->H || d->Wo != 2 * d->W || d->H < 1 || d->W < 1) return VK_ERR_UNSUPPORTED;
+  if (dsc->N != d->N || dsc->H != d->H || dsc->W != d->W || dsc->Ho != d->Ho || dsc->Wo != d->Wo || dsc->K != d->K) return VK_ERR_UNSUPPORTED;
+  const vk_src &a = d->src0, &b = dsc->src0;
+  if (d->src1.ptr || dsc->src1.ptr || a.up || b.up || a.scale || b.scale || !a.ptr || !b.ptr) return VK_ERR_UNSUPPORTED;
+  if (a.C != b.C) return VK_ERR_UNSUPPORTED;
+  const int C = a.C;
+  if (d->K < 64 || d->K % 64 || C < 32 || C % 32) return VK_ERR_UNSUPPORTED;
+  if (bnr && (!bnr->mask || !bnr->z || !bnr->sums)) return VK_ERR_UNSUPPORTED;
+  if ((size_t)d->N * d->H * d->W * C * 2 >= (1ull << 31) || (size_t)d->N * d->Ho * d->Wo * d->K * 2 >= (1ull << 32) ||
+      (size_t)d->K * C * 2 * 9 >= (1ull << 31))
+    return VK_ERR_UNSUPPORTED;
+  if (getenv("VK_NO_S2_TILE")) return VK_ERR_UNSUPPORTED;
+  HaloParams p;
+  p.s0 = HaloSrc{a.ptr, nullptr, nullptr, C, 0, 0, (uint32_t)((size_t)d->N * d->H * d->W * C * 2)};
+  p.s1 = HaloSrc{nullptr, nullptr, nullptr, 0, 0, 0, 0u};
+  p.w = w_halo;
+  p.w_bytes = (uint32_t)((size_t)d->K * 9 * C * 2);
+  p.y0 = y; p.y1 = nullptr; p.split = 0;
+  p.ld0 = d->K; p.ld1 = 0;
+  p.stats = nullptr;
+  p.N = d->N; p.H = d->Ho; p.W = d->Wo; p.K = d->K; p.C = C;
+  p.Hi = d->H; p.Wi = d->W;
+  p.flip = 0;
+  p.accumulate = bnr ? bnr->accumulate : accumulate;
+  p.pool2 = 0;
+  p.tiles_x = p.tiles_y = 0;
+  p.nchunks = C / 32;
+  p.stamps = nullptr;
+  p.kyn = 0; p.ksplit = 1;
+  p.slab_bytes = 0; p.slab = nullptr;
+  p.dbg = 0;
+  p.bnr_z = bnr ? bnr->z : nullptr;
+  p.bnr_scale = nullptr; p.bnr_shift = nullptr;
+  p.bnr_sums = bnr ? bnr->sums : nullptr;
+  p.bnr_mask = bnr ? bnr->mask : nullptr;
+  p.w2 = w_sc;
+  p.w2_bytes = (uint32_t)((size_t)d->K * C * 2);
+  p.x2 = b.ptr;
+  p.x2_bytes = p.s0.bytes;
+  const long tiles = (long)d->N * ((d->H + 7) / 8) * ((d->W + 15) / 16);
+  const bool wide = d->K % 128 == 0 && tiles * (d->K / 128) >= 256;
+  if (d->dtype == VK_BF16) return wide ? launch_s2dg<bf16_t, 128, true>(p, st) : launch_s2dg<bf16_t, 64, true>(p, st);
+  return wide ? launch_s2dg<f16_t, 128, true>(p, st) : launch_s2dg<f16_t, 64, true>(p, st);
+}
+
+}
+
+extern "C" int vk_conv_dgrad_s2sc(const vk_conv_desc* d, const void* w_halo, const vk_conv_desc* d_sc, const void* w_sc, void* y, int accumulate,
+                                  const vk_bnr* bnr, void* stream) {
+  VK_CHECK_ARG(d && d_sc && w_halo && w_sc && y, "vk_conv_dgrad_s2sc: null argument");
+  return vk::conv3x3_s2sc_dgrad_impl(d, w_halo, d_sc, w_sc, y, accumulate, bnr, (hipStream_t)stream);
+}
+
+extern "C" int vk_conv_fwd_s2sc(const vk_conv_desc* d, const void* w_halo, const vk_conv_desc* d_sc, const void* w_sc, void* z, void* z_sc,
+                                double* stats, double* stats_sc, void* stream) {
+  VK_CHECK_ARG(d && d_sc && w_halo && w_sc && z && z_sc && z != z_sc, "vk_conv_fwd_s2sc: null or aliased argument");
+  return vk::conv3x3_s2sc_impl(d, w_halo, d_sc, w_sc, z, z_sc, stats, stats_sc, (hipStream_t)stream);
 }
 
 extern "C" int vk_dec4_tail_eval(vk_dtype dtype, int N, int H, int W, const vk_src* src, const void* w1_pack, const float* scale1,
diff --git a/vickers-hardness-unet_amd/csrc/engine.hip b/vickers-hardness-unet_amd/csrc/engine.hip
--- a/vickers-hardness-unet_amd/csrc/engine.hip
+++ b/vickers-hardness-unet_amd/csrc/engine.hip
@@ -1148,7 +1148,24 @@
   for (BlockL& k : h->blocks) {
     ConvL& c1 = h->convs[k.conv1];
     ConvL& c2 = h->convs[k.conv2];
-    RET_IF(run_conv(h, c1, to_src(cur), null_src(), training, st));
+    bool sc_fused = false;
+    if (k.convd >= 0 && k.conv3 < 0 && k.stride == 2 && dt != VK_F32 && c1.halo_fwd && !h->convs[k.convd].pw && !h->convs[k.convd].halo_fwd &&
+        !(!training && h->splitk_bytes) && !getenv("VK_NO_S2SC_FWD")) {
+      ConvL& cd = h->convs[k.convd];
+      BnL& b1 = h->bns[c1.bn];
+      BnL& bd = h->bns[cd.bn];
+      const vk_conv_desc d1 = conv_desc(h, c1, to_src(cur), null_src()), dd = conv_desc(h, cd, to_src(cur), null_src());
+      const int rc = vk_conv_fwd_s2sc(&d1, fwd_weights(h, c1), &dd, fwd_weights(h, cd), c1.z, cd.z, training && !frozen(h, b1) ? b1.stats : nullptr,
+                                      training && !frozen(h, bd) ? bd.stats : nullptr, st);
+      if (rc == VK_OK) {
+        RET_IF(finalize_bn(h, b1, training, st));
+        RET_IF(finalize_bn(h, bd, training, st));
+        sc_fused = true;
+      } else if (rc != VK_ERR_UNSUPPORTED) {
+        return rc;
+      }
+    }
+    if (!sc_fused) RET_IF(run_conv(h, c1, to_src(cur), null_src(), training, st));
     RET_IF(run_conv(h, c2, to_src(bn_act(h, c1)), null_src(), training, st));
     ConvL& ct = k.conv3 >= 0 ? h->convs[k.conv3] : c2;
     if (k.conv3 >= 0) RET_IF(run_conv(h, ct, to_src(bn_act(h, c2)), null_src(), training, st));
@@ -1156,7 +1173,7 @@
     const size_t pixels = (size_t)N * k.Hout * k.Wout;
     if (k.convd >= 0) {
       ConvL& cd = h->convs[k.convd];
-      RET_IF(run_conv(h, cd, to_src(cur), null_src(), training, st));
+      if (!sc_fused) RET_IF(run_conv(h, cd, to_src(cur), null_src(), training, st));
       const BnL& bd = h->bns[cd.bn];
       RET_IF(vk_bn_add_relu(dt, pixels, k.C, ct.z, b2.scale, b2.shift, cd.z, bd.scale, bd.shift, k.out, st));
     } else {
@@ -1508,10 +1525,29 @@
     if (rc == VK_OK) { tail_fused = true; h->tail_prereduced[(size_t)bi - 1] = 1; }
     else if (rc != VK_ERR_UNSUPPORTED) return rc;
   }
-  if (into_gin && !tail_fused) RET_IF(conv_dgrad(h, c1, gin, nullptr, 0, 1, st));
+  bool sc_dgrad = false;
+  if (into_gin && k.convd >= 0 && k.stride == 2 && dt != VK_F32 && c1.halo_dg && !h->convs[k.convd].pw && !getenv("VK_NO_S2SC_DGRAD")) {
+    ConvL& cd = h->convs[k.convd];
+    const vk_conv_desc d1 = dgrad_desc(h, c1), dd = dgrad_desc(h, cd);
+    const bool want_tail = bi > 0 && k.C <= tail_maxc && !getenv("VK_NO_TAIL_BNR_FUSION");
+    vk_bnr r;
+    if (want_tail) {
+      BlockL& pb = h->blocks[bi - 1];
+      ConvL& pc2 = h->convs[pb.conv2];
+      r.z = pc2.z; r.scale = nullptr; r.shift = nullptr; r.sums = h->bns[pc2.bn].bsums; r.mask = pb.out; r.accumulate = 1;
+    }
+    const int rc = vk_conv_dgrad_s2sc(&d1, dgrad_weights(h, c1), &dd, dgrad_weights(h, cd), gin, 1, want_tail ? &r : nullptr, st);
+    if (rc == VK_OK) {
+      sc_dgrad = true;
+      if (want_tail) h->tail_prereduced[(size_t)bi - 1] = 1;
+    } else if (rc != VK_ERR_UNSUPPORTED) {
+      return rc;
+    }
+  }
+  if (into_gin && !tail_fused && !sc_dgrad) RET_IF(conv_dgrad(h, c1, gin, nullptr, 0, 1, st));
   if (k.convd >= 0) {
     ConvL& cd = h->convs[k.convd];
-    if (into_gin) RET_IF(conv_dgrad(h, cd, gin, nullptr, 0, 1, st));
+    if (into_gin && !sc_dgrad) RET_IF(conv_dgrad(h, cd, gin, nullptr, 0, 1, st));
     if (trains(h, c1.w_t)) RET_IF(conv_wgrad(h, c1, to_src(xin), null_src(), st));
     return trains(h, cd.w_t) ? conv_wgrad(h, cd, to_src(xin), null_src(), st) : VK_OK;
   }
```

Result: no change. 3060 (median of 6 runs) (+0.9%).
